# jenkinsm13/julia-spira

Measured on AMD Instinct MI355X. Metric: Msamples/sec at 1920x1080 spp=64 depth=8; fraction of HBM roofline, higher is better.
Workload: dtype f64

## Files before the change

include/spira_hip.h:

```cpp
#ifndef SPIRA_HIP_H
#define SPIRA_HIP_H

#include <stdint.h>

#ifdef __cplusplus
extern "C" {
#endif

#define SPIRA_ABI_VERSION 3

#define SPIRA_OK            0
#define SPIRA_E_INVALID    -1
#define SPIRA_E_NO_DEVICE  -2
#define SPIRA_E_HIP        -3
#define SPIRA_E_LIMIT      -4
#define SPIRA_E_UNSUPPORTED -5

#define SPIRA_SEM_MASK          0x0000000Fu
#define SPIRA_SEM_A             0x00000000u
#define SPIRA_SEM_CPU           0x00000001u
#define SPIRA_SEM_METAL         0x00000002u
#define SPIRA_SEM_HYBRID        0x00000003u
#define SPIRA_KERNEL_MASK       0x000000F0u
#define SPIRA_KERNEL_DEFAULT    0x00000000u
// ... 223 lines not shown
int spira_scene_radiance_f64(const spira_scene *scene, const double *rays6, uint32_t n_rays, const spira_radiance *rp,
                             double *sum_rgb, uint8_t *out_valid);
int spira_scene_radiance_device_f32(const spira_scene *scene, const float *d_rays6, uint32_t n_rays, const spira_radiance *rp,
                                    float *d_sum_rgb, uint8_t *d_out_valid, void *stream);
int spira_scene_radiance_device_f64(const spira_scene *scene, const double *d_rays6, uint32_t n_rays, const spira_radiance *rp,
                                    double *d_sum_rgb, uint8_t *d_out_valid, void *stream);

#define SPIRA_CAM_PINHOLE 0u
#define SPIRA_CAM_THIN_LENS 1u
#define SPIRA_CAM_ORTHO 2u
typedef struct spira_lens {
    uint32_t model, width, height, sample;
    uint64_t seed;
    uint32_t row0, rows;
    double   lens_radius;
} spira_lens;
int spira_camera_rays_f32(const float camera12[12], const spira_lens *lens, float *rays6);
int spira_camera_rays_f64(const double camera12[12], const spira_lens *lens, double *rays6);
int spira_camera_rays_device_f32(const float camera12[12], const spira_lens *lens, float *d_rays6, void *stream);
int spira_camera_rays_device_f64(const double camera12[12], const spira_lens *lens, double *d_rays6, void *stream);

typedef struct spira_gather_visible {
    uint32_t spp, sample0;
    uint64_t seed;
    uint32_t key0, flags;
    double   t_min, t_max;
} spira_gather_visible;
int spira_gather_rays_f32(const float *points6, uint32_t n_points, uint32_t sample, uint64_t seed, uint32_t key0, float *rays6);
int spira_gather_rays_f64(const double *points6, uint32_t n_points, uint32_t sample, uint64_t seed, uint32_t key0, double *rays6);
int spira_gather_rays_device_f32(const float *d_points6, uint32_t n_points, uint32_t sample, uint64_t seed, uint32_t key0, float *d_rays6, void *stream);
int spira_gather_rays_device_f64(const double *d_points6, uint32_t n_points, uint32_t sample, uint64_t seed, uint32_t key0, double *d_rays6, void *stream);
int spira_scene_gather_f32(const spira_scene *scene, const float *points6, uint32_t n_points, const spira_radiance *rp,
                           float *sum_rgb, uint8_t *out_valid);
int spira_scene_gather_f64(const spira_scene *scene, const double *points6, uint32_t n_points, const spira_radiance *rp,
                           double *sum_rgb, uint8_t *out_valid);
int spira_scene_gather_device_f32(const spira_scene *scene, const float *d_points6, uint32_t n_points, const spira_radiance *rp,
                                  float *d_sum_rgb, uint8_t *d_out_valid, void *stream);
int spira_scene_gather_device_f64(const spira_scene *scene, const double *d_points6, uint32_t n_points, const spira_radiance *rp,
                                  double *d_sum_rgb, uint8_t *d_out_valid, void *stream);
int spira_scene_gather_visible_f32(const spira_scene *scene, const float *points6, uint32_t n_points, const spira_gather_visible *gv,
                                   uint32_t *visible_u32, uint8_t *out_valid);
int spira_scene_gather_visible_f64(const spira_scene *scene, const double *points6, uint32_t n_points, const spira_gather_visible *gv,
                                   uint32_t *visible_u32, uint8_t *out_valid);
int spira_scene_gather_visible_device_f32(const spira_scene *scene, const float *d_points6, uint32_t n_points, const spira_gather_visible *gv,
                                          uint32_t *d_visible_u32, uint8_t *d_out_valid, void *stream);
int spira_scene_gather_visible_device_f64(const spira_scene *scene, const double *d_points6, uint32_t n_points, const spira_gather_visible *gv,
                                          uint32_t *d_visible_u32, uint8_t *d_out_valid, void *stream);

int spira_accumulate_f32(const float *spheres5, const float *materials8, const float *triangles10,
                         const float camera12[12], const spira_params *params, uint32_t sample0,
                         float *sum_rgb, uint32_t *rng_states);
int spira_accumulate_f64(const double *spheres5, const double *materials8, const double *triangles10,
                         const double camera12[12], const spira_params *params, uint32_t sample0,
                         double *sum_rgb, uint32_t *rng_states);
int spira_accumulate_device_f32(const float *spheres5, const float *materials8, const float *triangles10,
                                const float camera12[12], const spira_params *params, uint32_t sample0,
                                float *d_sum_rgb, uint32_t *d_rng_states, void *stream);
int spira_accumulate_device_f64(const double *spheres5, const double *materials8, const double *triangles10,
                                const double camera12[12], const spira_params *params, uint32_t sample0,
                                double *d_sum_rgb, uint32_t *d_rng_states, void *stream);

typedef struct spira_adaptive {
    uint32_t min_spp, batch_spp;
    double   tolerance, floor;
} spira_adaptive;
int spira_render_adaptive_f32(const float *spheres5, const float *materials8, const float *triangles10,
                              const float camera12[12], const spira_params *params, const spira_adaptive *adaptive,
                              float *out_hdr, float *out_img, uint32_t *out_spp, float *out_q);
int spira_render_adaptive_f64(const double *spheres5, const double *materials8, const double *triangles10,
                              const double camera12[12], const spira_params *params, const spira_adaptive *adaptive,
                              double *out_hdr, double *out_img, uint32_t *out_spp, double *out_q);
int spira_render_adaptive_scene_f32(const spira_scene *scene, const float camera12[12], const spira_params *params, const spira_adaptive *adaptive,
                                    float *out_hdr, float *out_img, uint32_t *out_spp, float *out_q);
int spira_render_adaptive_scene_f64(const spira_scene *scene, const double camera12[12], const spira_params *params, const spira_adaptive *adaptive,
                                    double *out_hdr, double *out_img, uint32_t *out_spp, double *out_q);
int spira_render_adaptive_scene_device_f32(const spira_scene *scene, const float camera12[12], const spira_params *params, const spira_adaptive *adaptive,
                                           float *d_out_hdr, float *d_out_img, uint32_t *d_out_spp, float *d_out_q, void *stream);
int spira_render_adaptive_scene_device_f64(const spira_scene *scene, const double camera12[12], const spira_params *params, const spira_adaptive *adaptive,
                                           double *d_out_hdr, double *d_out_img, uint32_t *d_out_spp, double *d_out_q, void *stream);
int spira_adaptive_converged_f32(const float sum3[3], float q, uint32_t n, double tolerance, double floor);
int spira_adaptive_converged_f64(const double sum3[3], double q, uint32_t n, double tolerance, double floor);

int spira_sky_pixel_f64(const double camera12[12], uint32_t width, uint32_t height, uint32_t i, uint32_t j, const double *spheres5, uint32_t n_spheres);

int spira_render_features_f32(const float *spheres5, const float *materials8, const float *triangles10,
                              const float camera12[12], const spira_params *params,
                              float *out_albedo, float *out_normal, float *out_depth);
int spira_render_features_f64(const double *spheres5, const double *materials8, const double *triangles10,
                              const double camera12[12], const spira_params *params,
                              double *out_albedo, double *out_normal, double *out_depth);
int spira_render_features_scene_f32(const spira_scene *scene, const float camera12[12], const spira_params *params,
                                    float *out_albedo, float *out_normal, float *out_depth);
int spira_render_features_scene_f64(const spira_scene *scene, const double camera12[12], const spira_params *params,
                                    double *out_albedo, double *out_normal, double *out_depth);
int spira_render_features_scene_device_f32(const spira_scene *scene, const float camera12[12], const spira_params *params,
                                           float *d_out_albedo, float *d_out_normal, float *d_out_depth, void *stream);
int spira_render_features_scene_device_f64(const spira_scene *scene, const double camera12[12], const spira_params *params,
                                           double *d_out_albedo, double *d_out_normal, double *d_out_depth, void *stream);

typedef struct spira_denoise {
    uint32_t width, height, iterations, post;
    double   sigma_l, sigma_z;
} spira_denoise;
int spira_denoise_f32(const float *color, const float *variance, const float *albedo, const float *normal, const float *depth,
                      const spira_denoise *dn, float *out_hdr, float *out_img);
int spira_denoise_f64(const double *color, const double *variance, const double *albedo, const double *normal, const double *depth,
                      const spira_denoise *dn, double *out_hdr, double *out_img);
int spira_denoise_device_f32(const float *d_color, const float *d_variance, const float *d_albedo, const float *d_normal, const float *d_depth,
                             const spira_denoise *dn, float *d_out_hdr, float *d_out_img, void *stream);
int spira_denoise_device_f64(const double *d_color, const double *d_variance, const double *d_albedo, const double *d_normal, const double *d_depth,
                             const spira_denoise *dn, double *d_out_hdr, double *d_out_img, void *stream);

int spira_trace_paths_f32(const float *spheres5, const float *materials8, const float *triangles10,
                          const float camera12[12], const spira_params *params, uint32_t n_paths,
                          const uint32_t *ijs, int *prims, float *ts, float *dirs, float *radiance);
int spira_trace_paths_f64(const double *spheres5, const double *materials8, const double *triangles10,
                          const double camera12[12], const spira_params *params, uint32_t n_paths,
                          const uint32_t *ijs, int *prims, double *ts, double *dirs, double *radiance);

int spira_tonemap_f32(float *values, uint64_t n, uint32_t post);

uint32_t spira_stripe_rows(uint32_t height, uint32_t stripe_h, uint32_t stripe_count, uint32_t stripe_rank);

#ifdef __cplusplus
}
#endif
#endif
```

julia-spira_amd/csrc/spira_device.h:

```cpp
#pragma once
#include <hip/hip_runtime.h>
#include <stdint.h>
#include <type_traits>
#include "spira_fastdiv.h"
#include "spira_sky.h"

namespace spira {

__device__ __forceinline__ float sqrt_rn(float x) { return __builtin_sqrtf(x); }
__device__ __forceinline__ double sqrt_rn(double x) { return __builtin_sqrt(x); }

constexpr int kBlock = 256;
#ifndef SPIRA_WAVES_F32
#define SPIRA_WAVES_F32 5
#endif
#ifndef SPIRA_WAVES_F64
#define SPIRA_WAVES_F64 4
#endif
#define SPIRA_WAVES_PER_SIMD(T) (sizeof(T) == 8 ? SPIRA_WAVES_F64 : SPIRA_WAVES_F32)
constexpr uint32_t kMaxTries = 64;

template <class T> struct Vec { T x, y, z; };

template <class T> __device__ __forceinline__ Vec<T> mk(T x, T y, T z) { Vec<T> r; r.x = x; r.y = y; r.z = z; return r; }
// ... 655 lines not shown
    asm volatile("" :: "v"(u0.x), "v"(u0.y), "v"(u0.z), "v"(u0.w), "v"(u1.x), "v"(u1.y), "v"(u1.z), "v"(u1.w), "v"(u2.x), "v"(u2.y), "v"(u2.z), "v"(u2.w) : "memory");
    if (do_tri) {
        float t_hi;
        const int cls = tri_screen_f32(u0, u1, u2, r, dx, dy, dz, t_hi);
        if (cls != 0) {
            w.c3 = w.c2; w.c2 = w.c1; w.c1 = w.c0; w.c0 = ti; ++w.nc;
            if (cls == 2) r.best = __builtin_fminf(r.best, t_hi);
        }
    }
    if (do_node) {
        uint32_t ih, lh;
        bvh8_node(n0, n1, n2, n3, n4, r, ih, lh);
        w.G = (n1.x << 8) | ih;
        w.tw = n1.y | (lh << 24);
        w.rank = n1.z;
    }
    return ((w.tw >> 24) != 0 || (w.G & 0xFFu) != 0 || w.sp > 0) ? kWalkOn : kWalkDone;
}

template <class T, int KL = 0>
__device__ __forceinline__ void bvh_closest_hit(const SceneLds<T> &sc, Vec<T> o, Vec<T> d, T t_min, T &closest, int &prim, uint32_t &slot, uint32_t *lds_stack = nullptr) {
    Bvh8Ray r; T t0;
    if (!bvh8_enter<T>(sc, o, d, closest, r, t0)) return;
    Bvh8Walk<T> w;
    bvh8_begin<T>(w, r, t0, t_min, sc.bvh_root[2].w);
    uint32_t stack[kBvhStackD - KL];
    const uint32_t lane = threadIdx.x & 63;
    const int base = (int)(sc.n_spheres + sc.n_triangles);
    while (bvh8_step<T, KL>(sc, w, r, o, d, t_min, base, closest, prim, slot, lds_stack, stack, lane)) {}
    while (w.nc) bvh8_resolve_one<T>(sc, w, r, o, d, t_min, base, closest, prim, slot);
}

template <class T, class P, bool TRI = true, bool CAM = false>
__device__ __forceinline__ void closest_hit_local(const SceneLds<T> &sc, Vec<T> o, Vec<T> d, T t_min, T &closest, int &prim, P &pol, const Pack4<T> *cam = nullptr) {
    closest = (T)INFINITY;
    prim = -1;
    const T a = dot(d, d);
    const T two_a = (T)2.0 * a;
    const T four_a = (T)4 * a;
    const RootDiv<T> over_2a = root_divisor<T>(two_a, pol);
    root_t_min<T>(t_min, pol);
    const Pack4<T> *sph = CAM ? cam : sc.sph;
    Pack4<T> c_next = sph[0];
#pragma unroll 2
    for (uint32_t s = 0; s < sc.n_spheres; ++s) {
        const Pack4<T> c = c_next;
        c_next = sph[s + 1 < sc.n_spheres ? s + 1 : s];
        Vec<T> oc; T cc;
        if (CAM) { oc = mk<T>(c.x, c.y, c.z); cc = c.w; }
        else {
            oc = o - mk<T>(c.x, c.y, c.z);
            cc = dot(oc, oc) - c.w;
        }
        T b = (T)2.0 * dot(oc, d);
        const T bb = b * b;
        T disc = bb - four_a * cc;
        if (!(disc < 0)) {
            root_operands<T>(bb, disc, pol);
            T sq = root_sqrt<T>(disc, pol);
            T root = root_over<T>(-b - sq, over_2a, pol);
            bool ok = !(root < t_min || root > closest);
            if (!ok && root < t_min) {
                root = root_over<T>(-b + sq, over_2a, pol);
                ok = !(root < t_min || root > closest);
            }
            if (ok) { closest = root; prim = (int)s; }
        }
    }
    if (TRI && sc.n_triangles) {
        Pack4<T> v0n = sc.tri[0], e1n = sc.tri[1], e2n = sc.tri[2];
#pragma unroll 2
        for (uint32_t i = 0; i < sc.n_triangles; ++i) {
            const Pack4<T> v0 = v0n, e1 = e1n, e2 = e2n;
            const uint32_t nx = i + 1 < sc.n_triangles ? i + 1 : i;
            v0n = sc.tri[3 * nx]; e1n = sc.tri[3 * nx + 1]; e2n = sc.tri[3 * nx + 2];
            T t;
            if (triangle_test<T>(v0, e1, e2, o, d, t_min, closest, t, pol)) {
                closest = t; prim = (int)(sc.n_spheres + i);
            }
        }
    }
}

template <class T>
__device__ __forceinline__ bool mesh_box_hit(const SceneLds<T> &sc, Vec<T> o, Vec<T> d, T closest) {
    const Vec<T> inv = mk<T>(rcp_fast(d.x), rcp_fast(d.y), rcp_fast(d.z));
    return box_entry<T>(sc.bvh_root[0], sc.bvh_root[1], o, inv, closest) >= (T)0;
}

template <class T>
__device__ __forceinline__ void closest_hit_local(const SceneLds<T> &sc, Vec<T> o, Vec<T> d, T t_min, T &closest, int &prim) {
    ExactDiv exact;
    closest_hit_local<T>(sc, o, d, t_min, closest, prim, exact);
}
template <class T, bool BVH, class P, bool TRI = true>
__device__ __forceinline__ int closest_hit(const SceneLds<T> &sc, Vec<T> o, Vec<T> d, T t_min, T &t_hit, uint32_t &slot, P &pol) {
    T closest; int prim;
    closest_hit_local<T, P, TRI>(sc, o, d, t_min, closest, prim, pol);
    slot = 0;
    if (BVH) bvh_closest_hit<T>(sc, o, d, t_min, closest, prim, slot);
    t_hit = closest;
    return prim;
}
template <class T, bool BVH>
__device__ __forceinline__ int closest_hit(const SceneLds<T> &sc, Vec<T> o, Vec<T> d, T t_min, T &t_hit, uint32_t &slot) {
    ExactDiv exact;
    return closest_hit<T, BVH>(sc, o, d, t_min, t_hit, slot, exact);
}

template <class T> __device__ __forceinline__ Vec<T> random_in_unit_sphere(const RngKey &k) {
    Vec<T> p = mk<T>(0, 0, 0);
    for (uint32_t t = 1; t <= kMaxTries; ++t) {
        T u0, u1, u2;
        rng3<T>(k, t, u0, u1, u2, (T)(1.0 / 1048576.0));
        Vec<T> q = mk<T>(u0, u1, u2) - mk<T>(1, 1, 1);
        if (dot(q, q) < (T)1.0) { p = q; break; }
    }
    return p;
}

enum : uint32_t { kDead = 0, kDiffuse = 1, kSpecRough = 2, kMirror = 3, kDielectric = 4 };
template <class T> struct Pending { Vec<T> v; T rough; uint32_t kind; };
struct SegInfo { int prim; bool alive; bool has_contrib; };

template <class T> struct ExtState {
    uint32_t flags;
    T bR, bG, bB;
};

template <class T> __device__ __forceinline__ T spd_lookup(const T *tab, int row, int i, T f) {
    const T *t = tab + row * kSpdN;
    return t[i] + (t[i + 1] - t[i]) * f;
}
template <class T>
__device__ __forceinline__ Vec<T> ext_wavelength(const SceneLds<T> &sc, uint32_t sA, uint32_t sB, uint32_t pixel, uint32_t sample, ExtState<T> &ext) {
    T xu, xv, u2;
    rng3<T>(rng_key(sA, sB, pixel, sample, 0), 0, xu, xv, u2);
    const T x = u2 * (T)(kSpdN - 1);
    int i = (int)x;
    i = i > kSpdN - 2 ? kSpdN - 2 : i;
    const T f = x - (T)i;
    ext.bR = spd_lookup<T>(sc.spd, 0, i, f); ext.bG = spd_lookup<T>(sc.spd, 1, i, f); ext.bB = spd_lookup<T>(sc.spd, 2, i, f);
    return mk<T>(spd_lookup<T>(sc.spd, 3, i, f), spd_lookup<T>(sc.spd, 4, i, f), spd_lookup<T>(sc.spd, 5, i, f));
}
template <class T> __device__ __forceinline__ T ext_uplift(const ExtState<T> &ext, const Vec<T> c) { return (c.x * ext.bR + c.y * ext.bG) + c.z * ext.bB; }

template <class T> __device__ __forceinline__ Vec<T> sky_term(const Vec<T> d, const Vec<T> beta) {
    T ts = (T)0.5 * (d.y + (T)1.0);
    Vec<T> sky = mk<T>(1.0, 1.0, 1.0) * ((T)1.0 - ts) + mk<T>((T)0.5, (T)0.7, (T)1.0) * ts;
    return mulv(beta, sky);
}
template <class T, bool EXT> __device__ __forceinline__ Vec<T> sky_term_x(const Vec<T> d, const Vec<T> beta, const ExtState<T> *ext) {
    if (EXT && (ext->flags & kExtSpectral)) {
        T ts = (T)0.5 * (d.y + (T)1.0);
        Vec<T> sky = mk<T>(1.0, 1.0, 1.0) * ((T)1.0 - ts) + mk<T>((T)0.5, (T)0.7, (T)1.0) * ts;
        return beta * ext_uplift<T>(*ext, sky);
    }
    return sky_term<T>(d, beta);
}

template <class T, bool BVH, bool TRI = true> __device__ __forceinline__ int material_of(const SceneLds<T> &sc, int prim, uint32_t slot) {
    if ((!TRI && !BVH) || prim < (int)sc.n_spheres) return sc.smat[prim];
    if (TRI && (!BVH || prim < (int)(sc.n_spheres + sc.n_triangles))) return sc.tmat[prim - (int)sc.n_spheres];
    return (int)Bits<T>::to_u32(sc.bvh_tris[3 * (size_t)slot + 1].w);
}

// ... 76 lines not shown
    int prim = closest_hit<T, BVH>(sc, o, d, (T)0.001, t, slot);
    info.prim = prim;
    t_out = prim >= 0 ? t : (T)0;
    if (prim < 0) {
        pend.kind = kDead; pend.rough = 0; pend.v = mk<T>(0, 0, 0);
        contrib = sky_term_x<T, EXT>(d, beta, ext);
        info.alive = false; info.has_contrib = true;
        return info;
    }
    const Vec<T> pos = o + d * t;
    info.has_contrib = shade_hit<T, BVH, EXT>(sc, pos, d, prim, slot, beta, scatter, contrib, pend, ext);
    info.alive = scatter;
    if (scatter) o = pos;
    return info;
}

template <class T, class P>
__device__ __forceinline__ Vec<T> segment_back(const Vec<T> pos, const Pending<T> &pend, const Vec<T> rnd, P &pol) {
    if (pend.kind == kDiffuse) return normalize((pend.v + rnd) - pos, pol);
    Vec<T> reflected = pend.v;
    if (pend.kind == kSpecRough) reflected = reflected + rnd * pend.rough;
    return normalize(reflected, pol);
}
template <class T>
__device__ __forceinline__ Vec<T> segment_back(const Vec<T> pos, const Pending<T> &pend, const Vec<T> rnd) {
    ExactDiv exact;
    return segment_back<T>(pos, pend, rnd, exact);
}

template <class T, bool BVH, bool EXT = false>
__device__ __forceinline__ SegInfo trace_segment(const SceneLds<T> &sc, const RenderConst<T> &rc, Vec<T> &o, Vec<T> &d,
                                                 Vec<T> &beta, uint32_t pixel, uint32_t sample, uint32_t bounce,
                                                 bool scatter, Vec<T> &contrib, T &t_out, const ExtState<T> *ext = nullptr) {
    Pending<T> pend;
    const Vec<T> d_in = d;
    SegInfo info = segment_front<T, BVH, EXT>(sc, o, d, beta, scatter, contrib, t_out, pend, ext);
    if (info.alive) {
        Vec<T> rnd = mk<T>(0, 0, 0);
        if (EXT && pend.kind == kDielectric) dielectric_resolve<T>(pend, d_in, rng_key(rc.sA, rc.sB, pixel, sample, bounce));
        if (pend.kind == kDiffuse || pend.kind == kSpecRough)
            rnd = random_in_unit_sphere<T>(rng_key(rc.sA, rc.sB, pixel, sample, bounce));
        d = segment_back<T>(o, pend, rnd);
    }
    return info;
}

template <class T, class P>
__device__ __forceinline__ void camera_ray(const RenderConst<T> &rc, uint32_t i, uint32_t j, uint32_t pixel, uint32_t sample,
                                           Vec<T> &o, Vec<T> &d, P &pol) {
    T xu, xv, unused;
    rng3<T>(rng_key(rc.sA, rc.sB, pixel, sample, 0), 0, xu, xv, unused);
    T u = ((T)(i - 1) + xu) / (T)(rc.width - 1);
    T v = ((T)(j - 1) + xv) / (T)(rc.height - 1);
    o = rc.cam_origin;
    d = normalize(((rc.cam_llc + rc.cam_hor * u) + rc.cam_ver * v) - o, pol);
}
template <class T>
__device__ __forceinline__ void camera_ray(const RenderConst<T> &rc, uint32_t i, uint32_t j, uint32_t pixel, uint32_t sample,
                                           Vec<T> &o, Vec<T> &d) {
    ExactDiv exact;
    camera_ray<T>(rc, i, j, pixel, sample, o, d, exact);
}
__device__ __forceinline__ float to_scalar(float x) { return __uint_as_float(__builtin_amdgcn_readfirstlane(__float_as_uint(x))); }
__device__ __forceinline__ double to_scalar(double x) {
    const uint32_t lo = __builtin_amdgcn_readfirstlane((uint32_t)__double2loint(x)), hi = __builtin_amdgcn_readfirstlane((uint32_t)__double2hiint(x));
    return __hiloint2double((int)hi, (int)lo);
}
template <class T> struct PixelDiv { Recip<T> w1, h1; };
template <class T> __device__ __forceinline__ PixelDiv<T> pixel_divisors(const RenderConst<T> &rc) {
    PixelDiv<T> p;
    p.w1 = recip_of((T)(rc.width - 1)); p.h1 = recip_of((T)(rc.height - 1));
    p.w1.d = to_scalar(p.w1.d); p.w1.r = to_scalar(p.w1.r); p.h1.d = to_scalar(p.h1.d); p.h1.r = to_scalar(p.h1.r);
    return p;
}
template <class T> __device__ __forceinline__ T pixel_quotient(T n, const Recip<T> &rc, ExactDiv &) { return n / rc.d; }
template <class T> __device__ __forceinline__ T pixel_quotient(T n, const Recip<T> &rc, SpecDiv &) { return quotient(n, rc); }
template <class T, class P>
__device__ __forceinline__ void camera_ray_lds(const RenderConst<T> &rc, const T *cam, const PixelDiv<T> &pd, uint32_t i, uint32_t j, uint32_t pixel, uint32_t sample,
                                               Vec<T> &o, Vec<T> &d, P &pol) {
    T xu, xv, unused;
    rng3<T>(rng_key(rc.sA, rc.sB, pixel, sample, 0), 0, xu, xv, unused);
    T u = pixel_quotient<T>((T)(i - 1) + xu, pd.w1, pol);
    T v = pixel_quotient<T>((T)(j - 1) + xv, pd.h1, pol);
    o = mk<T>(cam[0], cam[1], cam[2]);
    const Vec<T> llc = mk<T>(cam[3], cam[4], cam[5]), hor = mk<T>(cam[6], cam[7], cam[8]), ver = mk<T>(cam[9], cam[10], cam[11]);
    d = normalize(((llc + hor * u) + ver * v) - o, pol);
}

template <class T>
__device__ __forceinline__ void path_of(const RenderConst<T> &rc, uint32_t q, uint32_t pass, uint32_t &i, uint32_t &j,
                                        uint32_t &pixel, uint32_t &sample) {
    uint32_t slot = fastdiv(q, rc.fd_tile);
    uint32_t pl = q - slot * rc.tile_pixels;
    uint32_t lr = fastdiv(pl, rc.fd_width);
    uint32_t lx = pl - lr * rc.width;
    j = ref_row_j(rc, lr);
    i = lx + 1;
    pixel = (j - 1) * rc.width + lx;
    sample = rc.sample0 + pass * rc.slots + slot;
}

template <class T> struct RayQueue { Pack4<T> *A; Pack4<T> *B; Pack2<T> *C; };

struct Stats {
    unsigned long long segments, rays_enqueued, radiance_rmw, radiance_store, redone_waves, rays_parked;
    unsigned long long mesh_wave_trips, mesh_lane_trips;
    unsigned long long sky_pixels;
};

template <class T> struct BounceArgs {
    SceneGlobal<T> scene;
    RenderConst<T> rc;
    RayQueue<T> qin, qout;
    Pack3<T> *L;
    const uint32_t *cnt_in;
    uint32_t *cnt_out;
    uint32_t *blk_stats;
    uint32_t cap;
    Stats *stats;
    uint32_t bounce;
    uint32_t pass;
    uint32_t n_first;
};

__device__ __forceinline__ void wave_lds_sync() {
    __builtin_amdgcn_fence(__ATOMIC_RELEASE, "wavefront");
    __builtin_amdgcn_wave_barrier();
    __builtin_amdgcn_fence(__ATOMIC_ACQUIRE, "wavefront");
}

#ifndef SPIRA_RND_TAIL
#define SPIRA_RND_TAIL 1
#endif
#ifndef SPIRA_RND_INT
#define SPIRA_RND_INT 1
#endif
template <class T> constexpr bool kRndPacked = SPIRA_RND_INT && sizeof(T) == 8;

template <class T, bool PACKED = kRndPacked<T>> struct RndTry {
    Vec<T> c;
    __device__ __forceinline__ bool draw(const RngKey &k, uint32_t t) {
        T u0, u1, u2;
        rng3<T>(k, t, u0, u1, u2, (T)(1.0 / 1048576.0));
        c = mk<T>(u0, u1, u2) - mk<T>(1, 1, 1);
        return dot(c, c) < (T)1.0;
    }
    __device__ __forceinline__ void zero() { c = mk<T>(0, 0, 0); }
    __device__ __forceinline__ void store(Pack4<T> *slot) const { Pack4<T> w; w.x = c.x; w.y = c.y; w.z = c.z; w.w = 0; *slot = w; }
    static __device__ __forceinline__ Vec<T> load(const Pack4<T> *slot) { const Pack4<T> w = *slot; return mk<T>(w.x, w.y, w.z); }
};
template <class T> struct RndTry<T, true> {
    uint32_t a, b;
    __device__ __forceinline__ bool draw(const RngKey &k, uint32_t t) {
        a = mix32((k.hA + t * 0x9E3779B9u) ^ k.hBr);
        b = mix32(a + k.hB);
        const int32_t k0 = (int32_t)(a >> 11) - (1 << 20), k1 = (int32_t)(b >> 11) - (1 << 20);
        const int32_t k2 = (int32_t)(((a & 0x7FFu) << 10) | (b & 0x3FFu)) - (1 << 20);
        const uint64_t s = (uint64_t)((int64_t)k0 * k0) + (uint64_t)((int64_t)k1 * k1) + (uint64_t)((int64_t)k2 * k2);
        return s < (1ull << 40);
    }
    __device__ __forceinline__ void zero() { a = 0x80000400u; b = 0x80000000u; }
    __device__ __forceinline__ void store(Pack4<T> *slot) const { *reinterpret_cast<uint2 *>(slot) = make_uint2(a, b); }
    static __device__ __forceinline__ Vec<T> load(const Pack4<T> *slot) {
        const uint2 w = *reinterpret_cast<const uint2 *>(slot);
        const T s = (T)(1.0 / 1048576.0);
        const T u0 = (T)(w.x >> 11) * s, u1 = (T)(w.y >> 11) * s, u2 = (T)(((w.x & 0x7FFu) << 10) | (w.y & 0x3FFu)) * s;
// ... 145 lines not shown
                    q[r] |= 0x80000000u;
                } else if (!si.alive && !has_l) {
                    Pack3<T> l; l.x = 0; l.y = 0; l.z = 0;
                    a.L[qi] = l;
                    ++n_store;
                }
                want = (pend[r].kind == kDiffuse || pend[r].kind == kSpecRough);
                if (want) {
                    if (!FIRST) path_of<T>(rc, qi, a.pass, pi, pj, pixel, sample);
                    key = rng_key(rc.sA, rc.sB, pixel, sample, a.bounce);
                }
            }
            if (scatter) {
                const unsigned long long m = __ballot(want);
                if (want) {
                    ent[r] = n_list + __popcll(m & lt_mask);
                    uint32_t *kw = reinterpret_cast<uint32_t *>(&s_rnd[ent[r]]);
                    kw[0] = key.hA; kw[1] = key.hB;
                }
                n_list += (uint32_t)__popcll(m);
            }
        }
        if (!scatter) continue;
        wave_lds_sync();
        drain_unit_sphere_list<T>(s_rnd, n_list, lane);
        wave_lds_sync();
#pragma unroll
        for (int r = 0; r < R; ++r) {
            const bool alive = pend[r].kind != kDead;
            const unsigned long long m = __ballot(alive);
            if (alive) {
                Vec<T> rnd = mk<T>(0, 0, 0);
                if (pend[r].kind != kMirror) rnd = RndTry<T>::load(&s_rnd[ent[r]]);
                const Vec<T> nd = segment_back<T>(o[r], pend[r], rnd);
                const uint32_t dst = region + fill + __popcll(m & lt_mask);
                Pack4<T> A, B; Pack2<T> C;
                A.x = o[r].x; A.y = o[r].y; A.z = o[r].z; A.w = nd.x;
                B.x = nd.y; B.y = nd.z; B.z = beta[r].x; B.w = beta[r].y;
                C.x = beta[r].z; C.y = Bits<T>::from_u32(q[r]);
                a.qout.A[dst] = A; a.qout.B[dst] = B; a.qout.C[dst] = C;
            }
            fill += (uint32_t)__popcll(m);
        }
        wave_lds_sync();
    }
    for (int sft = 32; sft > 0; sft >>= 1) { n_rmw += __shfl_down(n_rmw, sft); n_seg += __shfl_down(n_seg, sft); n_store += __shfl_down(n_store, sft); }
    if (lane == 0) {
        if (scatter) a.cnt_out[wid] = fill;
        a.blk_stats[4 * wid] = n_seg;
        a.blk_stats[4 * wid + 1] = n_rmw;
        a.blk_stats[4 * wid + 2] = n_store;
        a.blk_stats[4 * wid + 3] = FIRST ? 0u : n_seg;
    }
}

template <class T> struct PathArgs {
    SceneGlobal<T> scene;
    RenderConst<T> rc;
    RayQueue<T> q[2];
    uint32_t *qref[2];
    uint2 *qkey[2];
    uint32_t cam_consts;
    Pack3<T> *L;
    uint32_t *blk_stats;
    uint32_t cap;
    uint32_t pass;
    uint32_t n_first;
    uint32_t dense_pct;
    Pack4<T> *mesh_list;
    uint32_t mesh_min_batch;
    uint32_t refill_free;
    uint32_t mesh_mode;
    uint32_t *mesh_count;
    uint32_t resume_k, resume_nw;
    uint32_t *redo;
    uint32_t redo_only;
    Stats *stats;
    Pack4<T> *accum;
    FastDiv fd_keff;
    uint32_t k_eff;
    uint32_t accum_first;
    uint32_t l_private;
    uint32_t sky_runs;
};

#ifndef SPIRA_RESOLVE_RUN
#define SPIRA_RESOLVE_RUN 4
#endif
__device__ __forceinline__ uint32_t owned_pixel(uint32_t w, uint32_t nw, uint32_t l) {
    constexpr uint32_t kRun = SPIRA_RESOLVE_RUN;
    static_assert(64 % kRun == 0, "a run length divides the wave");
    return ((l / kRun) * nw + w) * kRun + l % kRun;
}

template <class T>
__device__ __forceinline__ void resolve_pixel(Pack4<T> *accum, const Pack3<T> *L, uint32_t tile_pixels, uint32_t k_eff, bool first_pass, uint32_t p) {
    Pack4<T> acc;
    if (first_pass) { acc.x = 0; acc.y = 0; acc.z = 0; acc.w = 0; } else acc = accum[p];
    uint32_t s = 0;
    for (; s + 8 <= k_eff; s += 8) {
        Pack3<T> l[8];
#pragma unroll
        for (int k = 0; k < 8; ++k) l[k] = L[(size_t)(s + k) * tile_pixels + p];
#pragma unroll
        for (int k = 0; k < 8; ++k) { acc.x = acc.x + l[k].x; acc.y = acc.y + l[k].y; acc.z = acc.z + l[k].z; }
    }
    for (; s < k_eff; ++s) {
        const Pack3<T> l = L[(size_t)s * tile_pixels + p];
        acc.x = acc.x + l.x; acc.y = acc.y + l.y; acc.z = acc.z + l.z;
    }
    accum[p] = acc;
}
template <class T>
__device__ __forceinline__ void resolve_pixel_run(Pack4<T> *accum, const Pack3<T> *Lp, uint32_t k_eff, bool first_pass, uint32_t p) {
    constexpr uint32_t kRun = SPIRA_RESOLVE_RUN;
    Pack4<T> acc;
    if (first_pass) { acc.x = 0; acc.y = 0; acc.z = 0; acc.w = 0; } else acc = accum[p];
    uint32_t s = 0;
    for (; s + 8 <= k_eff; s += 8) {
        Pack3<T> l[8];
#pragma unroll
        for (int k = 0; k < 8; ++k) l[k] = Lp[(s + k) * kRun];
#pragma unroll
        for (int k = 0; k < 8; ++k) { acc.x = acc.x + l[k].x; acc.y = acc.y + l[k].y; acc.z = acc.z + l[k].z; }
    }
    for (; s < k_eff; ++s) {
        const Pack3<T> l = Lp[s * kRun];
        acc.x = acc.x + l.x; acc.y = acc.y + l.y; acc.z = acc.z + l.z;
    }
    accum[p] = acc;
}

__device__ __forceinline__ float pack_qref(uint32_t q, uint32_t, float) { return __uint_as_float(q); }
__device__ __forceinline__ double pack_qref(uint32_t q, uint32_t ref, double) { return __longlong_as_double((long long)((unsigned long long)q | ((unsigned long long)ref << 32))); }
__device__ __forceinline__ uint32_t unpack_q(float w) { return __float_as_uint(w); }
__device__ __forceinline__ uint32_t unpack_q(double w) { return (uint32_t)(unsigned long long)__double_as_longlong(w); }
__device__ __forceinline__ uint32_t unpack_ref(double w) { return (uint32_t)((unsigned long long)__double_as_longlong(w) >> 32); }

#ifdef SPIRA_MESH_STATS
__device__ unsigned long long g_mesh_dbg[32];
#define MESH_STAT(...) __VA_ARGS__
#else
#define MESH_STAT(...)
#endif

#ifndef SPIRA_CARRY_KEY
#define SPIRA_CARRY_KEY 1
#endif
#ifndef SPIRA_WAVES_B_F32
#define SPIRA_WAVES_B_F32 4
#endif
#ifndef SPIRA_WAVES_B_F64
#define SPIRA_WAVES_B_F64 SPIRA_WAVES_F64
#endif
#ifndef SPIRA_WAVES_PATH_F32
#define SPIRA_WAVES_PATH_F32 6
#endif
template <class T, int R, bool BVH, bool EXT, bool SPEC, int MODE = 0, bool TRI = true>
__global__ __launch_bounds__(kBlock, MODE == 2 ? (sizeof(T) == 8 ? SPIRA_WAVES_B_F64 : SPIRA_WAVES_B_F32) : (sizeof(T) == 4 ? SPIRA_WAVES_PATH_F32 : SPIRA_WAVES_F64)) void k_path(const PathArgs<T> a) {
    extern __shared__ __attribute__((aligned(32))) unsigned char lds_raw[];
    constexpr uint32_t WPB = kBlock / 64, SUB = 64 * R;
    constexpr bool kRefArray = sizeof(T) == 4;
    constexpr bool kCarry = SPIRA_CARRY_KEY && !BVH && !EXT;
    constexpr uint32_t kStageShift = 25, kRefMask = (1u << kStageShift) - 1u;
    const uint32_t lane = threadIdx.x & 63, wave = threadIdx.x >> 6;
    const uint32_t NW = gridDim.x * WPB, wid = blockIdx.x * WPB + wave;
    const RenderConst<T> &rc = a.rc;
    using Pol = typename std::conditional<SPEC, SpecDiv, ExactDiv>::type;
    Pol pol;
    if (!SPEC && a.redo_only) {
        uint32_t any = 0;
        for (uint32_t w = 0; w < WPB; ++w) any |= a.redo[blockIdx.x * WPB + w];
        if (!any) return;
    }
    T *cam_lds = reinterpret_cast<T *>(lds_raw + scene_lds_bytes<T>(a.scene.n_spheres, a.scene.n_materials, a.scene.n_triangles) + WPB * SUB * sizeof(Pack4<T>));
    if (threadIdx.x < 12) {
        const Vec<T> *cv = threadIdx.x < 3 ? &rc.cam_origin : (threadIdx.x < 6 ? &rc.cam_llc : (threadIdx.x < 9 ? &rc.cam_hor : &rc.cam_ver));
        const uint32_t cc = threadIdx.x % 3;
        cam_lds[threadIdx.x] = cc == 0 ? cv->x : (cc == 1 ? cv->y : cv->z);
    }
    Pack4<T> *cam_sph = reinterpret_cast<Pack4<T> *>(reinterpret_cast<unsigned char *>(cam_lds) + 128);
    constexpr bool kCam = !EXT;
    if (kCam && MODE != 2 && a.cam_consts)
        for (uint32_t i = threadIdx.x; i < a.scene.n_spheres; i += blockDim.x) {
            const T *sp = a.scene.spheres5 + 5 * (size_t)i;
            const Vec<T> oc = rc.cam_origin - mk<T>(sp[0], sp[1], sp[2]);
            Pack4<T> k; k.x = oc.x; k.y = oc.y; k.z = oc.z; k.w = dot(oc, oc) - sp[3] * sp[3];
            cam_sph[i] = k;
        }
    const SceneLds<T> sc = stage_scene<T>(a.scene, lds_raw);
    const PixelDiv<T> pix_div = pixel_divisors<T>(rc);
    if (!SPEC && a.redo_only) {
        if (!a.redo[wid]) return;
        if (lane == 0) atomicAdd(&a.stats->redone_waves, 1ull);
    }
    Pack4<T> *s_rnd = reinterpret_cast<Pack4<T> *>(lds_raw + scene_lds_bytes<T>(a.scene.n_spheres, a.scene.n_materials, a.scene.n_triangles)) + wave * SUB;
    constexpr uint32_t mesh_mode = BVH ? (uint32_t)MODE : 0u;
    const uint32_t kseg = mesh_mode == 2u ? a.resume_k : 1u;
    if (mesh_mode == 2u && wid * kseg >= a.resume_nw) return;
    const uint32_t region = wid * kseg * a.cap;
    const unsigned long long lt_mask = (1ull << lane) - 1ull;
    const uint32_t ref_base = sc.n_spheres + sc.n_triangles;
    const bool mixed = mesh_mode != 0u || rc.max_depth <= 128u;
    const uint32_t dense_pct = mixed ? a.dense_pct : 0u;
    const bool defer = mesh_mode != 0u || (BVH && mixed && a.mesh_list != nullptr);
    Pack4<T> *mlist = a.mesh_list + 3 * (size_t)region;
    uint32_t n_rmw = 0, n_store = 0, n_seg = 0, n_enq = 0, n_park = 0;
    uint32_t n_wtrips = 0, n_ltrips = 0;
    uint32_t n_in = 0;
    const bool own = !BVH && !EXT && !TRI && sizeof(T) == 8 && a.accum != nullptr;
    const uint32_t n_own = own ? 64u * a.k_eff : 0u;
    const uint32_t n_sub_first = own ? (n_own + SUB - 1) / SUB : (a.n_first + SUB - 1) / SUB;
    const bool priv = kCarry && own && a.l_private != 0;
    const uint32_t l_base = priv ? wid * n_own : 0u;
    constexpr bool kOwnT = !BVH && !EXT && !TRI && sizeof(T) == 8;
    uint32_t sky_mask = 0;
    uint32_t *sky_word = reinterpret_cast<uint32_t *>(cam_lds + 12) + wave;
    static_assert(12 * sizeof(T) + WPB * sizeof(uint32_t) <= 128 || !kOwnT, "a word per wave behind the camera");
    if constexpr (kOwnT) {
        if (own && a.sky_runs) {
            constexpr uint32_t kRun = SPIRA_RESOLVE_RUN, kRuns = 64 / kRun, kRowSlots = 64 / kRun;
            static_assert(kRun == 4 && 2 * 64 * sizeof(Pack3<T>) <= SUB * sizeof(Pack4<T>), "the run mask below is written for runs of 4; a row of terms fits the work list");
            {
                const uint32_t px = owned_pixel(wid, NW, lane);
                bool sky = false;
                if (px < rc.tile_pixels) {
                    uint32_t pi, pj, pixel, sample;
                    path_of<T>(rc, px, a.pass, pi, pj, pixel, sample);
                    sky = sky_pixel(cam_lds, rc.width, rc.height, pi, pj, a.scene.spheres5, a.scene.n_spheres);
                }
                unsigned long long b = __ballot(sky);
                b &= b >> 1; b &= b >> 2;
                for (uint32_t g = 0; g < kRuns; ++g) sky_mask |= (uint32_t)((b >> (kRun * g)) & 1ull) << g;
            }
            Pack3<T> *s_sky = reinterpret_cast<Pack3<T> *>(s_rnd);
            for (uint32_t m = sky_mask; m; m &= m - 1u) {
                const uint32_t g = (uint32_t)__builtin_ctz(m);
                const uint32_t px = owned_pixel(wid, NW, g * kRun + lane % kRun);
                uint32_t pi, pj, pixel, sample0;
                path_of<T>(rc, px, a.pass, pi, pj, pixel, sample0);
                Pack3<T> acc;
                acc.x = 0; acc.y = 0; acc.z = 0;
                if (!a.accum_first && lane < kRun) { const Pack4<T> a0 = a.accum[px]; acc.x = a0.x; acc.y = a0.y; acc.z = a0.z; }
                for (uint32_t s0 = 0; s0 < a.k_eff; s0 += kRowSlots) {
                    const uint32_t slot = s0 + lane / kRun;
                    if (slot < a.k_eff) {
                        Vec<T> o_, d_;
                        camera_ray_lds<T>(rc, cam_lds, pix_div, pi, pj, pixel, sample0 + slot, o_, d_, pol);
                        const Vec<T> c = sky_term_x<T, EXT>(d_, mk<T>(1, 1, 1), nullptr);
                        Pack3<T> l; l.x = c.x; l.y = c.y; l.z = c.z;
                        s_sky[lane] = l;
                        ++n_seg; ++n_store;
                    }
                    wave_lds_sync();
                    if (lane < kRun) {
                        const uint32_t n = a.k_eff - s0 < kRowSlots ? a.k_eff - s0 : kRowSlots;
                        for (uint32_t k = 0; k < n; ++k) { const Pack3<T> l = s_sky[k * kRun + lane]; acc.x = acc.x + l.x; acc.y = acc.y + l.y; acc.z = acc.z + l.z; }
                    }
                    wave_lds_sync();
                }
                if (lane < kRun) a.L[priv ? l_base + g * a.k_eff * kRun + lane : px] = acc;
            }
        }
        if (own) { if (lane == 0) *sky_word = sky_mask; wave_lds_sync(); }
    }

    auto park = [&](uint32_t slot_i, const Vec<T> o_, const Vec<T> d_, const Vec<T> beta_, T closest_, uint32_t q_, int prim_, uint32_t stage_hit) {
        Pack4<T> A, B, C;
        A.x = o_.x; A.y = o_.y; A.z = o_.z; A.w = d_.x;
        B.x = d_.y; B.y = d_.z; B.z = beta_.x; B.w = beta_.y;
        C.x = beta_.z; C.y = closest_; C.z = Bits<T>::from_u32(q_); C.w = Bits<T>::from_u32((uint32_t)(prim_ + 1) | (stage_hit << kStageShift));
        mlist[3 * (size_t)slot_i] = A; mlist[3 * (size_t)slot_i + 1] = B; mlist[3 * (size_t)slot_i + 2] = C;
    };
    uint32_t mfill = 0;
    constexpr int kMaxSeg = 16;
    uint32_t pfx[kMaxSeg + 1];
    bool segmented = false;
    {
        uint32_t cnt = 0;
        if (mesh_mode == 2u && lane < kseg && wid * kseg + lane < a.resume_nw) cnt = a.mesh_count[wid * kseg + lane];
        pfx[0] = 0;
#pragma unroll
        for (int j = 0; j < kMaxSeg; ++j) pfx[j + 1] = pfx[j] + (uint32_t)__builtin_amdgcn_readlane((int)cnt, j);
        if (mesh_mode == 2u) { mfill = pfx[kMaxSeg]; segmented = true; }
    }
    const uint32_t first_sub = own ? 0u : (mesh_mode == 1u ? (wid % a.resume_k) * (NW / a.resume_k) + wid / a.resume_k : wid);
    const uint32_t sub_step = own ? 1u : NW;
    MESH_STAT(unsigned long long dbg_t0 = __builtin_readcyclecounter(); unsigned long long dbg_sess = 0, dbg_walk = 0; uint32_t dbg_ns = 0, dbg_ws = 0, dbg_ls = 0, dbg_rf = 0, dbg_rays = 0, dbg_rounds = 0, dbg_ws1 = 0, dbg_ls1 = 0, dbg_h[4] = {0, 0, 0, 0};)
    for (uint32_t round = 0; ; ++round) {
        MESH_STAT(++dbg_rounds;)
        const bool first = mesh_mode != 2u && round == 0;
        const RayQueue<T> qin = a.q[(round + 1) & 1], qout = a.q[round & 1];
        const uint32_t *rin = a.qref[(round + 1) & 1];
        uint32_t *rout = a.qref[round & 1];
        const uint2 *kin = a.qkey[(round + 1) & 1];
        uint2 *kout = a.qkey[round & 1];
        const uint32_t limit = first ? (own ? n_own : a.n_first) : n_in;
        const uint32_t n_sub = first ? n_sub_first : (n_in + SUB - 1) / SUB;
        uint32_t fill = 0;
        for (uint32_t sub = first ? first_sub : 0u; sub < n_sub; sub += first ? sub_step : 1u) {
            if constexpr (kOwnT) if (own && first) {
                const uint32_t m = (uint32_t)__builtin_amdgcn_readfirstlane((int)*sky_word);
                const uint32_t r0 = fastdiv(sub * SUB / SPIRA_RESOLVE_RUN, a.fd_keff), r1 = fastdiv((sub * SUB + SUB - 1) / SPIRA_RESOLVE_RUN, a.fd_keff);
                if (r0 == r1 && ((m >> r0) & 1u)) continue;
            }
            Vec<T> o[R], beta[R];
            Pending<T> pend[R];
            ExtState<T> ex[R];
            uint32_t q[R], ent[R], stg[R], ref[R];
            uint32_t ka[R], kb[R];
            bool valid[R];
#pragma unroll
            for (int r = 0; r < R; ++r) {
                const uint32_t idx = sub * SUB + r * 64 + lane;
                valid[r] = false; stg[r] = round; ref[r] = 0; q[r] = 0; ka[r] = 0; kb[r] = 0;
                pend[r].kind = kDead; pend[r].rough = 0; pend[r].v = mk<T>(0, 0, 0);
                o[r] = mk<T>(0, 0, 0); beta[r] = mk<T>(1, 1, 1);
                bool parked = false; T park_t = 0; int park_prim = -1;
                uint32_t qf = idx;
                bool in = idx < limit;
                if (own && first) {
                    const uint32_t t = idx / SPIRA_RESOLVE_RUN, run = fastdiv(t, a.fd_keff);
                    const uint32_t px = owned_pixel(wid, NW, run * SPIRA_RESOLVE_RUN + idx % SPIRA_RESOLVE_RUN);
                    qf = (t - run * a.k_eff) * rc.tile_pixels + px;
                    in = in && px < rc.tile_pixels;
                    if constexpr (kOwnT) in = in && !((*sky_word >> run) & 1u);
                }
                const uint32_t ql = priv ? l_base + idx : qf;
                if (in) {
                    if (first) {
                        uint32_t pixel, sample, pi, pj;
                        Vec<T> d;
                        q[r] = ql;
                        path_of<T>(rc, qf, a.pass, pi, pj, pixel, sample);
                        if (kCarry) { ka[r] = mix32(rc.sA + pixel) ^ (sample << 8); kb[r] = mix32(rc.sB ^ pixel) + (sample << 8); }
                        camera_ray_lds<T>(rc, cam_lds, pix_div, pi, pj, pixel, sample, o[r], d, pol);
                        if (EXT) { ex[r].flags = rc.flags; if (rc.flags & kExtSpectral) beta[r] = ext_wavelength<T>(sc, rc.sA, rc.sB, pixel, sample, ex[r]); }
                        T t; uint32_t slot = 0;
                        int prim;
                        if (defer) {
                            if (kCam && a.cam_consts) closest_hit_local<T, Pol, TRI, true>(sc, o[r], d, (T)0.001, t, prim, pol, cam_sph);
                            else closest_hit_local<T, Pol, TRI>(sc, o[r], d, (T)0.001, t, prim, pol);
                            parked = mesh_box_hit<T>(sc, o[r], d, t);
                        } else if (kCam && !BVH && a.cam_consts) { closest_hit_local<T, Pol, TRI, true>(sc, o[r], d, (T)0.001, t, prim, pol, cam_sph); }
                        else prim = closest_hit<T, BVH, Pol, TRI>(sc, o[r], d, (T)0.001, t, slot, pol);
                        ++n_seg;
                        if (parked) { park_t = t; park_prim = prim; pend[r].v = d; }
                        else if (prim < 0) {
                            const Vec<T> c = sky_term_x<T, EXT>(d, beta[r], &ex[r]);
                            Pack3<T> l; l.x = c.x; l.y = c.y; l.z = c.z;
                            a.L[ql] = l;
                            ++n_store;
                        } else {
                            valid[r] = true;
                            o[r] = o[r] + d * t;
                            ref[r] = (BVH && prim >= (int)ref_base) ? ref_base + slot : (uint32_t)prim;
                            pend[r].v = d;
                        }
                    } else {
                        const Pack4<T> A = qin.A[region + idx], B = qin.B[region + idx];
                        const Pack2<T> C = qin.C[region + idx];
                        o[r] = mk<T>(A.x, A.y, A.z);
                        pend[r].v = mk<T>(A.w, B.x, B.y);
                        beta[r] = mk<T>(B.z, B.w, C.x);
                        q[r] = unpack_q(C.y);
                        uint32_t w;
                        if constexpr (kRefArray) w = rin[region + idx]; else w = unpack_ref(C.y);
                        if (mixed) { stg[r] = w >> kStageShift; ref[r] = w & kRefMask; } else ref[r] = w;
                        if (kCarry) { const uint2 k = kin[region + idx]; ka[r] = k.x; kb[r] = k.y; }
                        valid[r] = true;
                    }
                }
                if (defer && first) {
                    const unsigned long long mp = __ballot(parked);
                    if (parked) park(mfill + __popcll(mp & lt_mask), o[r], pend[r].v, beta[r], park_t, q[r], park_prim, 0u);
                    mfill += (uint32_t)__popcll(mp); n_park += (uint32_t)__popcll(mp);
                }
            }
            while (true) {
                uint32_t n_list = 0, n_valid = 0;
#pragma unroll
                for (int r = 0; r < R; ++r) {
                    bool want = false;
                    RngKey key;
                    const Vec<T> d = pend[r].v;
                    pend[r].kind = kDead;
                    if (valid[r]) {
                        uint32_t pixel = 0, sample = 0, pi, pj;
                        const bool scatter = stg[r] + 1 < rc.max_depth;
                        int prim = (int)ref[r]; uint32_t slot = 0;
                        if (BVH && ref[r] >= ref_base) { prim = (int)ref_base; slot = ref[r] - ref_base; }
                        const uint32_t qi = q[r] & 0x7FFFFFFFu;
                        const bool has_l = (q[r] >> 31) != 0;
                        if (EXT) {
                            path_of<T>(rc, qi, a.pass, pi, pj, pixel, sample);
                            ex[r].flags = rc.flags;
                            if (rc.flags & kExtSpectral) (void)ext_wavelength<T>(sc, rc.sA, rc.sB, pixel, sample, ex[r]);
                        }
                        Vec<T> contrib;
                        const bool has_contrib = shade_hit<T, BVH, EXT, Pol, TRI>(sc, o[r], d, prim, slot, beta[r], scatter, contrib, pend[r], &ex[r], pol);
                        if (has_contrib) {
                            Pack3<T> l; l.x = contrib.x; l.y = contrib.y; l.z = contrib.z;
                            if (has_l) { const Pack3<T> l0 = a.L[qi]; l.x = l0.x + contrib.x; l.y = l0.y + contrib.y; l.z = l0.z + contrib.z; ++n_rmw; }
                            else ++n_store;
                            a.L[qi] = l;
                            q[r] |= 0x80000000u;
                        } else if (!scatter && !has_l) {
                            Pack3<T> l; l.x = 0; l.y = 0; l.z = 0;
                            a.L[qi] = l;
                            ++n_store;
                        }
                        want = (pend[r].kind == kDiffuse || pend[r].kind == kSpecRough);
                        if (want || (EXT && pend[r].kind == kDielectric)) {
                            if (kCarry && mixed) {
                                key.hA = mix32(ka[r] ^ stg[r]); key.hB = mix32(kb[r] + stg[r]); key.hBr = (key.hB << 16) | (key.hB >> 16);
                            } else {
                                if (!EXT) path_of<T>(rc, qi, a.pass, pi, pj, pixel, sample);
                                key = rng_key(rc.sA, rc.sB, pixel, sample, stg[r]);
                            }
                            if (EXT && pend[r].kind == kDielectric) dielectric_resolve<T>(pend[r], d, key);
                        }
                    }
                    const unsigned long long mv = __ballot(pend[r].kind != kDead);
                    n_valid += (uint32_t)__popcll(mv);
                    const unsigned long long m = __ballot(want);
                    if (want) {
                        ent[r] = n_list + __popcll(m & lt_mask);
// ... 228 lines not shown
                        const Vec<T> hp = o_ + d_ * closest;
                        const uint32_t w_ = ((prim >= (int)ref_base) ? ref_base + slot : (uint32_t)prim) | (stage_hit << kStageShift);
                        const uint32_t dst = region + fill + __popcll(mh & lt_mask);
                        Pack4<T> A, B; Pack2<T> C;
                        A.x = hp.x; A.y = hp.y; A.z = hp.z; A.w = d_.x;
                        B.x = d_.y; B.y = d_.z; B.z = beta_.x; B.w = beta_.y;
                        C.x = beta_.z; C.y = pack_qref(q_, w_, (T)0);
                        qout.A[dst] = A; qout.B[dst] = B; qout.C[dst] = C;
                        if constexpr (kRefArray) rout[dst] = w_;
                    }
                }
                fill += (uint32_t)__popcll(mh);
                finished = false;
                const unsigned long long mf = __ballot(!walking);
                const uint32_t take = min((uint32_t)__popcll(mf), mfill - next);
                if (!walking && (uint32_t)__popcll(mf & lt_mask) < take) {
                    const uint32_t e = next + (uint32_t)__popcll(mf & lt_mask);
                    const Pack4<T> *ent = mlist + 3 * (size_t)e;
                    if (segmented) {
                        uint32_t seg = 0, off = e;
#pragma unroll
                        for (int j = 1; j < kMaxSeg; ++j) if (e >= pfx[j]) { seg = (uint32_t)j; off = e - pfx[j]; }
                        ent = a.mesh_list + 3 * ((size_t)(wid * kseg + seg) * a.cap + off);
                    }
                    const Pack4<T> A = ent[0], B = ent[1], C = ent[2];
                    o_ = mk<T>(A.x, A.y, A.z); d_ = mk<T>(A.w, B.x, B.y); beta_ = mk<T>(B.z, B.w, C.x);
                    closest = C.y;
                    q_ = Bits<T>::to_u32(C.z);
                    const uint32_t pw = Bits<T>::to_u32(C.w);
                    prim = (int)(pw & kRefMask) - 1;
                    stage_hit = pw >> kStageShift;
                    slot = 0;
                    T t0;
                    if (bvh8_enter<T>(sc, o_, d_, closest, ry, t0)) { bvh8_begin<T>(wk, ry, t0, (T)0.001, sc.bvh_root[2].w); walking = true; }
                    else finished = true;
                }
                next += take;
                if (!__any(walking)) { if (__any(finished)) continue; break; }
                const bool more = next < mfill;
                MESH_STAT(++dbg_rf; const unsigned long long dbg_w0 = __builtin_readcyclecounter();)
                uint32_t n_now = (uint32_t)__popcll(__ballot(walking));
                while (true) {
                    ++n_wtrips; n_ltrips += n_now;
                    MESH_STAT(++dbg_ws; { const uint32_t nl = (uint32_t)__popcll(__ballot(walking)); dbg_ls += nl; if (segmented) { ++dbg_ws1; dbg_ls1 += nl; } ++dbg_h[nl <= 8 ? 0 : (nl <= 24 ? 1 : (nl <= 48 ? 2 : 3))]; })
                    if (walking && !bvh8_step<T, kLdsStack>(sc, wk, ry, o_, d_, (T)0.001, (int)ref_base, closest, prim, slot, lstack, stack, lane)) { walking = false; finished = true; }
                    const uint32_t n_walk = (uint32_t)__popcll(__ballot(walking));
                    n_now = n_walk;
                    if (n_walk == 0 || (more && 64u - n_walk >= a.refill_free)) break;
                }

                MESH_STAT(dbg_walk += __builtin_readcyclecounter() - dbg_w0;)
            }
            }
            mfill = 0;
            segmented = false;
            MESH_STAT(dbg_sess += __builtin_readcyclecounter() - dbg_s0;)
        }
        n_in = fill;
        n_enq += fill;
        if (n_in == 0 && (mfill == 0 || mesh_mode == 1u)) break;
        __builtin_amdgcn_fence(__ATOMIC_RELEASE, "workgroup");
        __builtin_amdgcn_fence(__ATOMIC_ACQUIRE, "workgroup");
    }
    for (int sft = 32; sft > 0; sft >>= 1) { n_rmw += __shfl_down(n_rmw, sft); n_seg += __shfl_down(n_seg, sft); n_store += __shfl_down(n_store, sft); }
    const bool again = SPEC && __any(outside_window<T>(pol));
    if (own && !again && !(SPEC && a.redo_only == 2u)) {
        __builtin_amdgcn_fence(__ATOMIC_RELEASE, "workgroup");
        __builtin_amdgcn_fence(__ATOMIC_ACQUIRE, "workgroup");
        const uint32_t px = owned_pixel(wid, NW, lane);
        bool summed = false;
        if constexpr (kOwnT) sky_mask = (uint32_t)__builtin_amdgcn_readfirstlane((int)*sky_word);
        if constexpr (kOwnT) summed = ((sky_mask >> (lane / SPIRA_RESOLVE_RUN)) & 1u) != 0;
        if (summed) {
            const Pack3<T> l = a.L[priv ? l_base + (lane / SPIRA_RESOLVE_RUN) * a.k_eff * SPIRA_RESOLVE_RUN + lane % SPIRA_RESOLVE_RUN : px];
            Pack4<T> acc;
            if (a.accum_first) acc.w = 0; else acc = a.accum[px];
            acc.x = l.x; acc.y = l.y; acc.z = l.z;
            a.accum[px] = acc;
        } else if (px < rc.tile_pixels) {
            if (priv) resolve_pixel_run<T>(a.accum, a.L + l_base + (lane / SPIRA_RESOLVE_RUN) * a.k_eff * SPIRA_RESOLVE_RUN + lane % SPIRA_RESOLVE_RUN, a.k_eff, a.accum_first != 0, px);
            else resolve_pixel<T>(a.accum, a.L, rc.tile_pixels, a.k_eff, a.accum_first != 0, px);
        }
        const uint32_t seg = __shfl(n_seg, 0), rmw = __shfl(n_rmw, 0), sto = __shfl(n_store, 0);
        if (lane < 4) {
            unsigned long long *f = lane == 0 ? &a.stats->segments : (lane == 1 ? &a.stats->rays_enqueued : (lane == 2 ? &a.stats->radiance_rmw : &a.stats->radiance_store));
            atomicAdd(f, (unsigned long long)(lane == 0 ? seg : (lane == 1 ? n_enq : (lane == 2 ? rmw : sto))));
        }
        if constexpr (kOwnT) if (lane == 4 && sky_mask) atomicAdd(&a.stats->sky_pixels, (unsigned long long)(SPIRA_RESOLVE_RUN * __popc(sky_mask)));
    }
    MESH_STAT(if (lane == 0) { unsigned long long *g = g_mesh_dbg + (mesh_mode == 2u ? 16 : 0);
                               atomicAdd(&g[0], __builtin_readcyclecounter() - dbg_t0); atomicAdd(&g[1], dbg_sess); atomicAdd(&g[2], (unsigned long long)dbg_ns);
                               atomicAdd(&g[3], (unsigned long long)dbg_ws); atomicAdd(&g[4], (unsigned long long)dbg_ls); atomicAdd(&g[5], (unsigned long long)dbg_rf);
                               atomicAdd(&g[6], (unsigned long long)dbg_rays); atomicAdd(&g[7], (unsigned long long)dbg_rounds); atomicAdd(&g[9], dbg_walk); atomicAdd(&g[10], 1ull); atomicAdd(&g[11], (unsigned long long)dbg_ws1); atomicAdd(&g[12], (unsigned long long)dbg_ls1);
                               atomicAdd(&g[8], (unsigned long long)dbg_h[0]); atomicAdd(&g[13], (unsigned long long)dbg_h[1]); atomicAdd(&g[14], (unsigned long long)dbg_h[2]); atomicAdd(&g[15], (unsigned long long)dbg_h[3]); })
    if (lane == 0) {
        if (mesh_mode == 2u) {
            const uint32_t row = 4 * wid * kseg;
            a.blk_stats[row] += n_seg; a.blk_stats[row + 1] += n_rmw; a.blk_stats[row + 2] += n_store; a.blk_stats[row + 3] += n_enq;
        } else {
            a.blk_stats[4 * wid] = n_seg;
            a.blk_stats[4 * wid + 1] = n_rmw;
            a.blk_stats[4 * wid + 2] = n_store;
            a.blk_stats[4 * wid + 3] = n_enq;
            if (mesh_mode == 1u) a.mesh_count[wid] = mfill;
        }
        if (SPEC) a.redo[wid] = again ? 1u : 0u;
        if (BVH && n_park && !again && !(SPEC && a.redo_only == 2u)) atomicAdd(&a.stats->rays_parked, (unsigned long long)n_park);
        if (BVH && mesh_mode != 1u && n_wtrips && !again && !(SPEC && a.redo_only == 2u)) { atomicAdd(&a.stats->mesh_wave_trips, (unsigned long long)n_wtrips); atomicAdd(&a.stats->mesh_lane_trips, (unsigned long long)n_ltrips); }
    }
}

template <class T, bool BVH, bool EXT>
__global__ __launch_bounds__(kBlock) void k_mega(const BounceArgs<T> a) {
    extern __shared__ __attribute__((aligned(32))) unsigned char lds_raw[];
    const SceneLds<T> sc = stage_scene<T>(a.scene, lds_raw);
    const RenderConst<T> &rc = a.rc;
    unsigned long long nseg = 0;
    const uint32_t stride = gridDim.x * kBlock;
    uint32_t idx = blockIdx.x * kBlock + threadIdx.x;
    bool fresh = true;
    uint32_t pixel = 0, sample = 0, b = 0;
    Vec<T> o = mk<T>(0, 0, 0), d = mk<T>(0, 0, 1), beta = mk<T>(1, 1, 1), Lacc = mk<T>(0, 0, 0);
    ExtState<T> ex; ex.flags = rc.flags; ex.bR = 0; ex.bG = 0; ex.bB = 0;
    while (idx < a.n_first) {
        if (fresh) {
            uint32_t pi, pj;
            path_of<T>(rc, idx, a.pass, pi, pj, pixel, sample);
            camera_ray<T>(rc, pi, pj, pixel, sample, o, d);
            beta = mk<T>(1, 1, 1); Lacc = mk<T>(0, 0, 0); b = 0;
            if (EXT && (rc.flags & kExtSpectral)) beta = ext_wavelength<T>(sc, rc.sA, rc.sB, pixel, sample, ex);
            fresh = false;
        }
        Vec<T> contrib; T t_hit;
        SegInfo si = trace_segment<T, BVH, EXT>(sc, rc, o, d, beta, pixel, sample, b, b + 1 < rc.max_depth, contrib, t_hit, &ex);
        ++nseg;
        if (b == 0) { if (si.has_contrib) Lacc = contrib; }
        else if (si.has_contrib) Lacc = Lacc + contrib;
        ++b;
        if (!si.alive || b == rc.max_depth) {
            Pack3<T> l; l.x = Lacc.x; l.y = Lacc.y; l.z = Lacc.z;
            a.L[idx] = l;
            idx += stride;
            fresh = true;
        }
    }
    for (int sft = 32; sft > 0; sft >>= 1) nseg += __shfl_down(nseg, sft);
    if ((threadIdx.x & 63) == 0 && nseg) atomicAdd(&a.stats->segments, nseg);
}

template <class T, bool BVH, bool EXT>
__global__ __launch_bounds__(64) void k_trace(const BounceArgs<T> a, const uint32_t *ijs, uint32_t n_paths, int *prims, T *ts,
                                              T *dirs, T *radiance) {
    extern __shared__ __attribute__((aligned(32))) unsigned char lds_raw[];
    const SceneLds<T> sc = stage_scene<T>(a.scene, lds_raw);
    const RenderConst<T> &rc = a.rc;
    uint32_t p = blockIdx.x * blockDim.x + threadIdx.x;
    if (p >= n_paths) return;
    uint32_t i = ijs[3 * p], j = ijs[3 * p + 1], sample = ijs[3 * p + 2];
    uint32_t pixel = (j - 1) * rc.width + (i - 1);
    Vec<T> o, d, beta = mk<T>(1, 1, 1), Lacc = mk<T>(0, 0, 0);
    camera_ray<T>(rc, i, j, pixel, sample, o, d);
    ExtState<T> ex; ex.flags = rc.flags; ex.bR = 0; ex.bG = 0; ex.bB = 0;
    if (EXT && (rc.flags & kExtSpectral)) beta = ext_wavelength<T>(sc, rc.sA, rc.sB, pixel, sample, ex);
    for (uint32_t b = 0; b < rc.max_depth; ++b) {
        Vec<T> contrib; T t_hit;
        Vec<T> dir_in = d;
        SegInfo si = trace_segment<T, BVH, EXT>(sc, rc, o, d, beta, pixel, sample, b, b + 1 < rc.max_depth, contrib, t_hit, &ex);
        size_t k = (size_t)p * rc.max_depth + b;
        prims[k] = si.prim; ts[k] = t_hit;
        dirs[3 * k] = dir_in.x; dirs[3 * k + 1] = dir_in.y; dirs[3 * k + 2] = dir_in.z;
        if (b == 0) { if (si.has_contrib) Lacc = contrib; }
// ... 756 lines not shown
```

julia-spira_amd/csrc/spira_hip.hip:

```cpp
#include <hip/hip_runtime.h>
#include <sys/mman.h>
#include <rccl/rccl.h>
#include <dlfcn.h>

#include <algorithm>
#include <atomic>
#include <chrono>
#include <cmath>
#include <cstdio>
#include <cstdlib>
#include <cstring>
#include <condition_variable>
#include <mutex>
#include <new>
#include <string>
#include <thread>
#include <type_traits>
#include <vector>

#include "../../include/spira_hip.h"
#include "../../include/spira_spd.h"
#include "spira_device.h"
#include "spira_bvh.h"
#include "spira_validate.h"
// ... 584 lines not shown
                std::memcpy(pieces[i].dst, (const char *)c.h_stage + pieces[i].off, pieces[i].len);
            }
        };
        std::vector<std::thread> thr;
        for (int t = 1; t < n_thr; ++t) thr.emplace_back(mover, t);
        mover(0);
        for (auto &t : thr) t.join();
        for (hipError_t e : errs) if (e != hipSuccess) return e;
        return hipSuccess;
    }
};

int copy_out(Ctx &c, hipStream_t st, void *const dst[2], const void *const src[2], size_t bytes_each) {
    const size_t kChunk = (size_t)std::max<uint32_t>(1, env_u32("SPIRA_STAGE_CHUNK_MB", 8)) << 20, kMinStaged = 4u << 20, kMaxStaged = 512u << 20;
    const int n_out = (dst[0] ? 1 : 0) + (dst[1] ? 1 : 0);
    if (!n_out) return 0;
    const size_t total = bytes_each * (size_t)n_out;
    if (bytes_each < kMinStaged || total > kMaxStaged || !stage_reserve(c, total)) {
        for (int k = 0; k < 2; ++k) if (dst[k]) HIP_TRY(hipMemcpyAsync(dst[k], src[k], bytes_each, hipMemcpyDeviceToHost, st));
        return 0;
    }
    StagedCopy sc(c);
    for (int k = 0; k < 2; ++k)
        for (size_t o = 0; dst[k] && o < bytes_each; o += kChunk)
            HIP_TRY(sc.stage(st, (char *)dst[k] + o, (const char *)src[k] + o, std::min(kChunk, bytes_each - o)));
    const hipError_t e = sc.move();
    if (e != hipSuccess) return fail(SPIRA_E_HIP, std::string("copy_out: ") + hipGetErrorString(e));
    return 0;
}

template <class T>
int acquire_scene(Ctx &c, hipStream_t st, const spira_scene *h, const T *spheres5, const T *materials8, const T *triangles10,
                  const spira_params *p, spira::SceneGlobal<T> &g, bool reuse = false) {
    if (h) { scene_pointers<T>(h->store, g); return 0; }
    if (reuse) { scene_pointers<T>(c.scene, g); return 0; }
    const uint32_t nt = triangles10 ? p->n_triangles : 0;
    if (int rc = scene_upload<T>(c.scene, st, c.have_done ? c.ev_done : nullptr, spheres5, materials8, triangles10, p->n_spheres, p->n_materials, nt)) return rc;
    scene_pointers<T>(c.scene, g);
    return 0;
}

template <class T>
int attach_spd(Ctx &c, hipStream_t st, uint32_t flags, spira::SceneGlobal<T> &g) {
    g.spd = nullptr;
    if (!(flags & SPIRA_EXT_SPECTRAL)) return 0;
    DevBuf &b = sizeof(T) == 4 ? c.spd32 : c.spd64;
    if (!b.p) {
        static_assert(SPIRA_SPD_N == spira::kSpdN && SPIRA_SPD_ROWS == spira::kSpdRows, "SPD table shape");
        T host[SPIRA_SPD_ROWS * SPIRA_SPD_N];
        for (int r = 0; r < SPIRA_SPD_ROWS; ++r)
            for (int i = 0; i < SPIRA_SPD_N; ++i) host[r * SPIRA_SPD_N + i] = (T)spira_spd_table[r][i];
        if (int rc = b.ensure(sizeof host)) return rc;
        HIP_TRY(hipMemcpy(b.p, host, sizeof host, hipMemcpyHostToDevice));
    }
    (void)st;
    g.spd = (const T *)b.p;
    return 0;
}
template <class T>
int attach_spd(Ctx &c, hipStream_t st, const spira_params *p, spira::SceneGlobal<T> &g) { return attach_spd<T>(c, st, p->flags, g); }

template <class T>
int check_handle(const spira_scene *h) {
    if (!h || h->magic != kSceneMagic) return fail(SPIRA_E_INVALID, "scene handle is NULL or was destroyed");
    if (h->prec != (int)sizeof(T)) return fail(SPIRA_E_INVALID, "scene handle was created in the other precision");
    if (h->device != tl_device) return fail(SPIRA_E_INVALID, "scene handle belongs to another device (spira_set_device)");
    return 0;
}

spira::Knobs read_knobs() {
    spira::Knobs k;
    k.batch_rays = env_u32("SPIRA_BATCH_RAYS", k.batch_rays);
    k.R = env_u32("SPIRA_R", k.R);
    k.blocks_per_cu = env_u32("SPIRA_BLOCKS_PER_CU", 0);
    k.defer_mesh = env_u32("SPIRA_DEFER_MESH", 1); k.mesh_two_pass = env_u32("SPIRA_MESH_TWO_PASS", 1);
    k.fused_resolve = env_u32("SPIRA_FUSED_RESOLVE", 1); k.private_l = env_u32("SPIRA_PRIVATE_L", 1);
    k.spec_div = env_u32("SPIRA_SPEC_DIV", 1);
    k.dense_pct = std::min<uint32_t>(env_u32("SPIRA_DENSE_PCT", 70), 100);
    k.mesh_min_batch = std::max<uint32_t>(1, env_u32("SPIRA_MESH_MIN_BATCH", 128));
    k.mesh_refill = std::min<uint32_t>(64, std::max<uint32_t>(1, env_u32("SPIRA_MESH_REFILL", 16)));
    k.mesh_fat_waves_per_cu = env_u32("SPIRA_MESH_FAT_WAVES_PER_CU", 16);
    k.cam_consts = env_u32("SPIRA_CAM_CONSTS", 1);
    k.sky_runs = env_u32("SPIRA_SKY_RUNS", 1);
    return k;
}
template <class T>
spira::PlanIn plan_input(const Ctx &c, const spira_params *p, uint32_t rows, uint32_t nt_scene, bool progressive, bool caller_rng, bool out_on_device) {
    spira::PlanIn in;
    in.width = p->width; in.rows = rows; in.spp = p->spp; in.max_depth = p->max_depth; in.flags = p->flags; in.batch_rays = p->batch_rays;
    in.n_triangles = nt_scene; in.num_cus = (uint32_t)c.num_cus;
    in.progressive = progressive; in.caller_rng = caller_rng; in.out_on_device = out_on_device;
    in.prec = sizeof(T); in.block = spira::kBlock; in.waves_per_simd = SPIRA_WAVES_PER_SIMD(T); in.carry_key = SPIRA_CARRY_KEY;
    in.pack4 = sizeof(spira::Pack4<T>); in.pack3 = sizeof(spira::Pack3<T>); in.pack2 = sizeof(spira::Pack2<T>);
    in.k = read_knobs();
    return in;
}

int ensure_workspaces(Ctx &c, const spira::Workspace &w) {
    for (int i = 0; i < 2; ++i) {
        if (int rc = c.qA[i].ensure(w.queue4)) return rc;
        if (int rc = c.qB[i].ensure(w.queue4)) return rc;
        if (int rc = c.qC[i].ensure(w.queue2)) return rc;
        if (int rc = c.qR[i].ensure(w.q_ref)) return rc;
        if (int rc = c.qK[i].ensure(w.q_key)) return rc;
        if (int rc = c.qX[i].ensure(w.q_x)) return rc;
    }
    const struct { DevBuf &b; uint64_t bytes; } rest[] = {
        {c.mesh_list, w.mesh_list}, {c.mesh_count, w.mesh_count}, {c.redo, w.redo}, {c.blkstats, w.blkstats}, {c.L, w.L}, {c.counts, w.counts},
        {c.stats, sizeof(spira::Stats)}, {c.accum, w.accum}, {c.out_tmp, w.out_tmp}, {c.rng, w.rng},
        {c.hyb_state, w.hyb_state}, {c.hyb_mat, w.hyb_mat}, {c.hyb_flags, w.hyb_flags}};
    for (const auto &r : rest)
        if (int rc = r.b.ensure(r.bytes)) return rc;
    return 0;
}

template <class T>
int verify_path_args(const Ctx &c, const spira::PathArgs<T> &a, uint32_t first_launch_blocks) {
    using P4 = spira::Pack4<T>;
    using P2 = spira::Pack2<T>;
    spira::PathLaunch l;
    l.blocks = first_launch_blocks; l.cap = a.cap; l.n_first = a.n_first; l.k_eff = a.k_eff;
    l.tile_pixels = a.rc.tile_pixels; l.max_depth = a.rc.max_depth; l.flags = a.rc.flags; l.n_lds_triangles = a.scene.n_triangles;
    l.mesh_mode = a.mesh_mode; l.resume_k = a.resume_k; l.resume_nw = a.resume_nw;
    l.mesh = a.scene.n_bvh_tris != 0; l.pixel_owning = a.accum != nullptr; l.l_private = a.l_private != 0;
    l.prec = sizeof(T); l.wpb = spira::kBlock / 64; l.carry_key = SPIRA_CARRY_KEY;
    const spira::PathNeed need = spira::path_need(l);
    const uint64_t nw = need.nw, n = need.packets;
    auto covers = [](const DevBuf &b, const void *ptr, uint64_t bytes) { return ptr == b.p && b.p != nullptr && b.cap >= bytes; };
    const char *bad = need.fits ? nullptr : "the pass does not fit its queue regions";
    if (a.rc.max_depth > 1 || l.mesh)
        for (int i = 0; i < 2 && !bad; ++i) {
            if (!covers(c.qA[i], a.q[i].A, n * sizeof(P4)) || !covers(c.qB[i], a.q[i].B, n * sizeof(P4)) || !covers(c.qC[i], a.q[i].C, n * sizeof(P2))) bad = "hit queues";
            else if (sizeof(T) == 4 && !covers(c.qR[i], a.qref[i], n * sizeof(uint32_t))) bad = "hit reference arrays";
            else if (!l.mesh && !covers(c.qK[i], a.qkey[i], n * sizeof(uint2))) bad = "carried RNG keys";
        }
    if (!bad && a.mesh_list && !covers(c.mesh_list, a.mesh_list, 3 * n * sizeof(P4))) bad = "mesh lists";
    if (!bad && a.mesh_mode != 0 && (!a.mesh_list || !covers(c.mesh_count, a.mesh_count, nw * sizeof(uint32_t)) || !need.resume_ok)) bad = "parked-ray counts of a two-launch mesh pass";
    if (!bad && a.redo && !covers(c.redo, a.redo, nw * sizeof(uint32_t))) bad = "redo flags";
    if (!bad && !covers(c.blkstats, a.blk_stats, nw * 4 * sizeof(uint32_t))) bad = "per-wave statistics";
    if (!bad && !covers(c.L, a.L, need.l_entries * sizeof(spira::Pack3<T>))) bad = "per-path radiance";
    if (!bad && !covers(c.stats, a.stats, sizeof(spira::Stats))) bad = "counters";
    if (!bad && a.accum && (!covers(c.accum, a.accum, (uint64_t)a.rc.tile_pixels * sizeof(P4)) || !need.owning_ok)) bad = "pixel-owning pass";
    if (!bad && a.l_private && !need.private_ok) bad = "wave-private radiance blocks";
    if (bad) return fail(SPIRA_E_LIMIT, std::string("internal: a workspace is smaller than the launch needs (") + bad + ")");
    return 0;
}

template <class T>
int validate_call(const spira_scene *h, const T *spheres5, const T *materials8, const T *triangles10, const T *camera12, const spira_params *p,
                  const T *out_hdr, const T *out_img, bool progressive, uint32_t sample0, const uint32_t *rng_states, uint32_t *rows) {
    if (!p) return fail(SPIRA_E_INVALID, "params is NULL");
    const uint32_t nt = triangles10 ? p->n_triangles : 0;
    if (h) { if (int rc = check_handle<T>(h)) return rc; }
    else if (int rc = validate_scene<T>(spheres5, materials8, triangles10, p->n_spheres, p->n_materials, nt)) return rc;
    if (int rc = validate_params(camera12, p, h ? h->store.nt : nt, rows)) return rc;
    if (!out_hdr && !out_img) return fail(SPIRA_E_INVALID, "both outputs are NULL");
    const char *msg = nullptr;
    if (int rc = spira::sample_range_check(progressive, sample0, p->spp, &msg)) return fail(rc, msg);
    if (progressive && (p->flags & SPIRA_SEM_MASK) == SPIRA_SEM_HYBRID) return fail(SPIRA_E_UNSUPPORTED, "SPIRA_SEM_HYBRID has no accumulate entry (its image is a mean of tone-mapped samples)");
    if (progressive && (p->flags & SPIRA_SEM_MASK) == SPIRA_SEM_METAL && sample0 > 0 && !rng_states)
        return fail(SPIRA_E_INVALID, "SPIRA_SEM_METAL with sample0 > 0 needs rng_states (the LCG states the previous call left); "
                                     "without them every call would replay the samples of the first");
    return 0;
}

template <class T> struct Call {
    Ctx &c;
    hipStream_t st;
    const spira_params *p;
    const spira::Plan &plan;
    spira::BounceArgs<T> a{};
    size_t lds = 0;
    int spec = 0;
    bool progressive = false, profile = false;
    uint32_t sample0 = 0, *d_rng = nullptr;
    uint64_t launches = 0, metal_launches = 0;
    using P4 = spira::Pack4<T>;
    using P2 = spira::Pack2<T>;
    P4 *accum() const { return (P4 *)c.accum.p; }
    spira::Stats *stats() const { return (spira::Stats *)c.stats.p; }
    uint32_t *redo() const { return (uint32_t *)c.redo.p; }
    spira::RayQueue<T> queue(int i) const { return {(P4 *)c.qA[i].p, (P4 *)c.qB[i].p, (P2 *)c.qC[i].p}; }
    dim3 block() const { return dim3(spira::kBlock); }
    int resume() const { return progressive ? (sample0 > 0 ? 3 : 1) : 0; }
};

template <class T>
int enqueue_hybrid(Call<T> &k) {
    Ctx &c = k.c;
    const spira_params *p = k.p;
    const spira::Workspace &w = k.plan.ws;
    const uint32_t P = (uint32_t)k.plan.tile_pixels, hblocks = k.plan.blocks(P);
    HIP_TRY(hipMemsetAsync(c.hyb_flags.p, 0, w.hyb_flags, k.st));
    HIP_TRY(hipMemsetAsync(c.accum.p, 0, w.accum, k.st));
    HIP_TRY(hipMemsetAsync(c.hyb_mat.p, 0, w.hyb_mat, k.st));
    HIP_TRY(hipMemsetAsync(c.hyb_state.p, 0, w.hyb_state, k.st));
    hipLaunchKernelGGL(spira::k_hybrid_init, dim3(hblocks), k.block(), 0, k.st, (uint32_t *)c.rng.p, P, k.a.rc.sA, k.a.rc.sB);
    spira::HybridArgs<T> ha{};
    ha.scene = k.a.scene; ha.rc = k.a.rc; ha.state = (T *)c.hyb_state.p; ha.mat = (uint32_t *)c.hyb_mat.p; ha.rng = (uint32_t *)c.rng.p;
    ha.accum = k.accum(); ha.flags = (uint32_t *)c.hyb_flags.p; ha.stats = k.stats();
    for (uint32_t smp = 1; smp <= p->spp; ++smp)
        for (uint32_t ph = 0; ph <= p->max_depth; ++ph) {
            ha.sample = smp; ha.phase = ph;
            if (int rc = launch_lds(spira::k_hybrid<T>, dim3(hblocks), k.block(), k.lds, k.st, ha)) return rc;
        }
    k.launches += 1 + (uint64_t)p->spp * (p->max_depth + 1);
    return 0;
}

template <class T>
int enqueue_metal_wavefront(Call<T> &k) {
    Ctx &c = k.c;
    const spira::Plan &plan = k.plan;
    const dim3 grid(plan.G_metal);
    spira::MetalArgs<T> ma{};
    ma.scene = k.a.scene; ma.rc = k.a.rc;
    ma.ppw = plan.ppw;
    for (int i = 0; i < 2; ++i) { ma.q[i] = k.queue(i); ma.qx[i] = (uint2 *)c.qX[i].p; }
    if (!k.d_rng) k.d_rng = (uint32_t *)c.rng.p;
    ma.L = k.a.L; ma.accum = k.accum(); ma.rng_states = k.d_rng; ma.blk_stats = (uint32_t *)c.blkstats.p;
    ma.resume = k.resume();
    if (int rc = profile_events(c, c.ev_used + 2)) return rc;
    HIP_TRY(hipEventRecord(c.ev_pool[c.ev_used++], k.st));
    ma.stats = k.stats(); ma.redo = nullptr; ma.redo_only = 0;
    if (k.spec) {
        ma.redo = k.redo();
        ma.redo_only = k.spec == 2 ? 2 : 0;
        if (int rc = launch_lds(spira::k_path_metal<T, 2, true>, grid, k.block(), k.lds, k.st, ma)) return rc;
        ma.redo_only = 1;
        ++k.launches;
    }
    if (int rc = plan.R == 2 ? launch_lds(spira::k_path_metal<T, 2, false>, grid, k.block(), k.lds, k.st, ma)
                             : launch_lds(spira::k_path_metal<T, 1, false>, grid, k.block(), k.lds, k.st, ma)) return rc;
    HIP_TRY(hipEventRecord(c.ev_pool[c.ev_used++], k.st));
    hipLaunchKernelGGL(spira::k_fold_stats, dim3(1), dim3(64), 0, k.st, (const uint32_t *)c.blkstats.p, plan.G_metal * plan.wpb, k.stats());
    k.launches += 2;
    k.metal_launches = 1;
    return 0;
}

template <class T>
int enqueue_metal(Call<T> &k) {
    const dim3 grid(k.plan.blocks(k.plan.tile_pixels));
    k.a.pass = 0; k.a.n_first = (uint32_t)k.plan.tile_pixels;
    if (k.spec) {
        if (int rc = launch_lds(spira::k_variant_metal<T, true>, grid, k.block(), k.lds, k.st, k.a, k.accum(), k.d_rng, k.resume(), k.redo(), k.spec == 2 ? 2 : 0)) return rc;
        if (int rc = launch_lds(spira::k_variant_metal<T, false>, grid, k.block(), k.lds, k.st, k.a, k.accum(), k.d_rng, k.resume(), k.redo(), 1)) return rc;
    } else if (int rc = launch_lds(spira::k_variant_metal<T, false>, grid, k.block(), k.lds, k.st, k.a, k.accum(), k.d_rng, k.resume(), (uint32_t *)nullptr, 0))
        return rc;
    k.launches += k.spec ? 2 : 1;
    return 0;
}

template <class T>
int enqueue_cpu_pass(Call<T> &k) {
    const dim3 grid(k.plan.blocks(k.a.n_first));
    if (k.spec) {
        if (int rc = launch_lds(spira::k_variant_cpu<T, true>, grid, k.block(), k.lds, k.st, k.a, k.redo(), k.spec == 2 ? 2 : 0)) return rc;
        if (int rc = launch_lds(spira::k_variant_cpu<T, false>, grid, k.block(), k.lds, k.st, k.a, k.redo(), 1)) return rc;
    } else if (int rc = launch_lds(spira::k_variant_cpu<T, false>, grid, k.block(), k.lds, k.st, k.a, (uint32_t *)nullptr, 0))
        return rc;
    k.launches += k.spec ? 2 : 1;
    return 0;
}

template <class T>
int enqueue_mega_pass(Call<T> &k) {
    const dim3 grid(k.plan.blocks(k.a.n_first));
    const bool ext = (k.p->flags & (SPIRA_EXT_DIELECTRIC | SPIRA_EXT_SPECTRAL)) != 0;
    int rc;
    if (k.a.scene.n_bvh_tris) rc = ext ? launch_lds(spira::k_mega<T, true, true>, grid, k.block(), k.lds, k.st, k.a) : launch_lds(spira::k_mega<T, true, false>, grid, k.block(), k.lds, k.st, k.a);
    else rc = ext ? launch_lds(spira::k_mega<T, false, true>, grid, k.block(), k.lds, k.st, k.a) : launch_lds(spira::k_mega<T, false, false>, grid, k.block(), k.lds, k.st, k.a);
    ++k.launches;
    return rc;
}

template <class T>
int enqueue_path_pass(Call<T> &k, uint32_t *stat_rows) {
    using P4 = typename Call<T>::P4;
    Ctx &c = k.c;
    const spira::Plan &plan = k.plan;
    const spira::Knobs &kn = plan.in.k;
    spira::PathArgs<T> pa{};
    pa.scene = k.a.scene; pa.rc = k.a.rc; pa.L = k.a.L; pa.pass = k.a.pass; pa.n_first = k.a.n_first;
    pa.dense_pct = kn.dense_pct;
    pa.mesh_list = plan.defer_mesh ? (P4 *)c.mesh_list.p : nullptr;
    const spira::Geometry g = plan.geometry(pa.n_first);
    const uint32_t G = g.G;
    pa.cap = g.cap;
    *stat_rows = G * plan.wpb;
    for (int i = 0; i < 2; ++i) {
        pa.q[i] = k.queue(i);
        pa.qref[i] = (uint32_t *)c.qR[i].p;
        pa.qkey[i] = (uint2 *)c.qK[i].p;
    }
    pa.blk_stats = (uint32_t *)c.blkstats.p;
    pa.stats = k.stats();
    if (k.spec) pa.redo = k.redo();
    pa.mesh_mode = 0; pa.mesh_count = nullptr; pa.resume_k = 1; pa.resume_nw = 0;
    pa.mesh_min_batch = kn.mesh_min_batch;
    pa.refill_free = kn.mesh_refill;
    size_t lds_a = k.lds + (size_t)plan.wpb * plan.sub * sizeof(P4) + 128;
    pa.cam_consts = (kn.cam_consts && pa.scene.n_spheres && lds_a + (size_t)pa.scene.n_spheres * sizeof(P4) <= (size_t)160 * 1024) ? 1u : 0u;
    if (pa.cam_consts) lds_a += (size_t)pa.scene.n_spheres * sizeof(P4);
    if (plan.two_pass) {
        pa.mesh_mode = 1; pa.mesh_count = (uint32_t *)c.mesh_count.p;
        pa.resume_nw = G * plan.wpb; pa.resume_k = plan.fat_k(pa.resume_nw);
    }
    if (plan.fused) {
        pa.accum = k.accum(); pa.k_eff = plan.k_eff(pa.pass); pa.fd_keff = spira::fastdiv_make(pa.k_eff);
        pa.accum_first = (pa.pass == 0 && !k.progressive) ? 1u : 0u;
        pa.l_private = plan.l_private ? 1u : 0u;
        pa.sky_runs = plan.sky_runs ? 1u : 0u;
    }
    if (int rc = verify_path_args<T>(c, pa, G)) return rc;
    HIP_TRY(hipEventRecord(c.ev_pool[c.ev_used++], k.st));
    if (int rc = launch_path<T>((int)plan.R, dim3(G), lds_a, k.st, pa, k.spec)) return rc;
    k.launches += k.spec ? 2 : 1;
    if (pa.mesh_mode == 1) {
        if (c.ev_mid.size() <= c.ev_mid_used) {
            hipEvent_t e;
            HIP_TRY(hipEventCreate(&e));
            c.ev_mid.push_back(e); c.ev_mid_end.push_back(0);
        }
        HIP_TRY(hipEventRecord(c.ev_mid[c.ev_mid_used], k.st));
        c.ev_mid_end[c.ev_mid_used++] = c.ev_used;
        spira::PathArgs<T> pb = pa;
        pb.mesh_mode = 2; pb.n_first = 0;
        const uint32_t nwb = pa.resume_nw / pa.resume_k;
        if (int rc = launch_path_resume_entry<T>((int)plan.R, dim3((nwb + plan.wpb - 1) / plan.wpb), lds_a, k.st, pb)) return rc;
        ++k.launches;
    }
    HIP_TRY(hipEventRecord(c.ev_pool[c.ev_used++], k.st));
    return 0;
}

template <class T>
int enqueue_bounce_pass(Call<T> &k, uint32_t *stat_rows) {
    using P4 = typename Call<T>::P4;
    Ctx &c = k.c;
    const spira::Plan &plan = k.plan;
    const spira::Geometry g = plan.geometry(k.a.n_first);
    const size_t nw = (size_t)g.G * plan.wpb;
    k.a.cap = g.cap;
    *stat_rows = k.p->max_depth * g.G * plan.wpb;
    for (uint32_t b = 0; b < k.p->max_depth; ++b) {
        k.a.bounce = b;
        k.a.qout = k.queue(b & 1);
        k.a.qin = k.queue((b & 1) ^ 1);
        k.a.cnt_in = (const uint32_t *)c.counts.p + (size_t)b * nw;
        k.a.cnt_out = (uint32_t *)c.counts.p + (size_t)(b + 1) * nw;
        k.a.blk_stats = (uint32_t *)c.blkstats.p + (size_t)b * nw * 4;
        if (k.profile) HIP_TRY(hipEventRecord(c.ev_pool[c.ev_used++], k.st));
        const size_t lds_b = k.lds + (size_t)plan.wpb * plan.sub * sizeof(P4);
        if (int rc = b == 0 ? launch_bounce<T, true>((int)plan.R, dim3(g.G), lds_b, k.st, k.a) : launch_bounce<T, false>((int)plan.R, dim3(g.G), lds_b, k.st, k.a)) return rc;
        if (k.profile) HIP_TRY(hipEventRecord(c.ev_pool[c.ev_used++], k.st));
        ++k.launches;
    }
    return 0;
}

template <class T>
void enqueue_resolve(Call<T> &k, uint32_t stat_rows) {
    const spira::Plan &plan = k.plan;
    hipLaunchKernelGGL((spira::k_resolve<T>), dim3(plan.blocks(plan.tile_pixels)), k.block(), 0, k.st, k.accum(), (const spira::Pack3<T> *)k.c.L.p,
                       (uint32_t)plan.tile_pixels, plan.k_eff(k.a.pass), (k.a.pass == 0 && !k.progressive) ? 1 : 0,
                       stat_rows ? (const uint32_t *)k.c.blkstats.p : (const uint32_t *)nullptr, stat_rows, k.stats());
    ++k.launches;
}

template <class T>
void enqueue_finalize(Call<T> &k, T *d_hdr, T *d_img) {
    using P4 = typename Call<T>::P4;
    const spira::Plan &plan = k.plan;
    const dim3 grid(plan.blocks(plan.tile_pixels));
    if (k.progressive)
        hipLaunchKernelGGL((spira::k_finalize<T>), grid, k.block(), 0, k.st, (const P4 *)k.accum(), (uint32_t)plan.tile_pixels, 1u, (uint32_t)SPIRA_POST_NONE, d_hdr, (T *)nullptr);
    else
        hipLaunchKernelGGL((spira::k_finalize<T>), grid, k.block(), 0, k.st, (const P4 *)k.accum(), (uint32_t)plan.tile_pixels, k.p->spp,
                           (k.p->flags & SPIRA_SEM_MASK) == SPIRA_SEM_HYBRID ? (uint32_t)SPIRA_POST_NONE : (k.p->flags & SPIRA_POST_MASK), d_hdr, d_img);
    ++k.launches;
}

template <class T>
int prepare_path_call(Call<T> &k, const spira_scene *h, const T *spheres5, const T *materials8, const T *triangles10, const T *camera12, uint32_t rows, bool reuse_scene) {
    Ctx &c = k.c;
    if (int rc = acquire_scene<T>(c, k.st, h, spheres5, materials8, triangles10, k.p, k.a.scene, reuse_scene)) return rc;
    if (int rc = attach_spd<T>(c, k.st, k.p, k.a.scene)) return rc;
    k.spec = k.plan.spec((h ? h->store.moderate : c.scene.moderate) && spira::camera_scale_moderate<T>(camera12));
    fill_const<T>(k.a.rc, camera12, k.p, rows, k.plan.slots);
    if (!fastdiv_selfcheck(k.a.rc.tile_pixels, (uint32_t)k.plan.batch) || !fastdiv_selfcheck(k.a.rc.width, k.a.rc.tile_pixels) ||
        !fastdiv_selfcheck(k.a.rc.stripe_h ? k.a.rc.stripe_h : 1, rows))
        return fail(SPIRA_E_LIMIT, "internal: fast division self-check failed");
    k.a.L = (spira::Pack3<T> *)c.L.p;
    k.a.stats = k.stats();
    k.lds = spira::scene_lds_bytes<T>(k.a.scene.n_spheres, k.a.scene.n_materials, k.a.scene.n_triangles);
    return 0;
}
// ... 2242 lines not shown
int spira_render_multi_scene_f64(const spira_scene *scene, const double cam[12], const spira_params *p, int n_devices, double *out_hdr, double *out_img) {
    if (!scene) return fail(SPIRA_E_INVALID, "scene handle is NULL or was destroyed");
    return render_multi_impl<double>(scene, nullptr, nullptr, nullptr, cam, p, n_devices, out_hdr, out_img);
}
int spira_scene_destroy(spira_scene *scene) {
    if (!scene) return 0;
    if (scene->magic != kSceneMagic) return fail(SPIRA_E_INVALID, "scene handle was already destroyed");
    for (int d = kMaxDevices - 1; d >= 0; --d) {
        spira_scene *h = d ? scene->replica[d] : scene;
        if (!h) continue;
        if (hipSetDevice(h->device) != hipSuccess) return fail(SPIRA_E_HIP, "hipSetDevice failed");
        h->store.release();
        h->magic = 0;
        delete h;
    }
    (void)hipSetDevice(tl_device);
    return 0;
}
int spira_scene_update_f32(spira_scene *scene, const float *spheres5, const float *materials8, const float *triangles10) {
    return scene_update_entry<float>(scene, spheres5, materials8, triangles10, nullptr, false, nullptr);
}
int spira_scene_update_f64(spira_scene *scene, const double *spheres5, const double *materials8, const double *triangles10) {
    return scene_update_entry<double>(scene, spheres5, materials8, triangles10, nullptr, false, nullptr);
}
int spira_scene_update_device_f32(spira_scene *scene, const float *d_triangles10, void *stream) {
    return scene_update_entry<float>(scene, nullptr, nullptr, nullptr, d_triangles10, true, stream);
}
int spira_scene_update_device_f64(spira_scene *scene, const double *d_triangles10, void *stream) {
    return scene_update_entry<double>(scene, nullptr, nullptr, nullptr, d_triangles10, true, stream);
}
int spira_scene_rebuild_f32(spira_scene *scene, const float *triangles10) { return scene_rebuild_entry<float>(scene, triangles10, nullptr, false, nullptr); }
int spira_scene_rebuild_f64(spira_scene *scene, const double *triangles10) { return scene_rebuild_entry<double>(scene, triangles10, nullptr, false, nullptr); }
int spira_scene_rebuild_device_f32(spira_scene *scene, const float *d_triangles10, void *stream) { return scene_rebuild_entry<float>(scene, nullptr, d_triangles10, true, stream); }
int spira_scene_rebuild_device_f64(spira_scene *scene, const double *d_triangles10, void *stream) { return scene_rebuild_entry<double>(scene, nullptr, d_triangles10, true, stream); }
int spira_render_scene_f32(const spira_scene *scene, const float cam[12], const spira_params *p, float *out_hdr, float *out_img) {
    if (!scene) return fail(SPIRA_E_INVALID, "scene handle is NULL or was destroyed");
    return render_entry<float>(scene, nullptr, nullptr, nullptr, cam, p, out_hdr, out_img, false, nullptr);
}
int spira_render_scene_f64(const spira_scene *scene, const double cam[12], const spira_params *p, double *out_hdr, double *out_img) {
    if (!scene) return fail(SPIRA_E_INVALID, "scene handle is NULL or was destroyed");
    return render_entry<double>(scene, nullptr, nullptr, nullptr, cam, p, out_hdr, out_img, false, nullptr);
}
int spira_render_scene_device_f32(const spira_scene *scene, const float cam[12], const spira_params *p, float *d_hdr, float *d_img, void *stream) {
    if (!scene) return fail(SPIRA_E_INVALID, "scene handle is NULL or was destroyed");
    return render_entry<float>(scene, nullptr, nullptr, nullptr, cam, p, d_hdr, d_img, true, stream);
}
int spira_render_scene_device_f64(const spira_scene *scene, const double cam[12], const spira_params *p, double *d_hdr, double *d_img, void *stream) {
    if (!scene) return fail(SPIRA_E_INVALID, "scene handle is NULL or was destroyed");
    return render_entry<double>(scene, nullptr, nullptr, nullptr, cam, p, d_hdr, d_img, true, stream);
}

int spira_render_adaptive_f32(const float *s, const float *m, const float *t, const float cam[12], const spira_params *p, const spira_adaptive *adaptive,
                              float *out_hdr, float *out_img, uint32_t *out_spp, float *out_q) {
    return render_adaptive_entry<float>(nullptr, s, m, t, cam, p, adaptive, out_hdr, out_img, out_spp, out_q, false, nullptr);
}
int spira_render_adaptive_f64(const double *s, const double *m, const double *t, const double cam[12], const spira_params *p, const spira_adaptive *adaptive,
                              double *out_hdr, double *out_img, uint32_t *out_spp, double *out_q) {
    return render_adaptive_entry<double>(nullptr, s, m, t, cam, p, adaptive, out_hdr, out_img, out_spp, out_q, false, nullptr);
}
int spira_render_adaptive_scene_f32(const spira_scene *scene, const float cam[12], const spira_params *p, const spira_adaptive *adaptive,
                                    float *out_hdr, float *out_img, uint32_t *out_spp, float *out_q) {
    if (!scene) return fail(SPIRA_E_INVALID, "scene handle is NULL or was destroyed");
    return render_adaptive_entry<float>(scene, nullptr, nullptr, nullptr, cam, p, adaptive, out_hdr, out_img, out_spp, out_q, false, nullptr);
}
int spira_render_adaptive_scene_f64(const spira_scene *scene, const double cam[12], const spira_params *p, const spira_adaptive *adaptive,
                                    double *out_hdr, double *out_img, uint32_t *out_spp, double *out_q) {
    if (!scene) return fail(SPIRA_E_INVALID, "scene handle is NULL or was destroyed");
    return render_adaptive_entry<double>(scene, nullptr, nullptr, nullptr, cam, p, adaptive, out_hdr, out_img, out_spp, out_q, false, nullptr);
}
int spira_render_adaptive_scene_device_f32(const spira_scene *scene, const float cam[12], const spira_params *p, const spira_adaptive *adaptive,
                                           float *d_hdr, float *d_img, uint32_t *d_spp, float *d_q, void *stream) {
    if (!scene) return fail(SPIRA_E_INVALID, "scene handle is NULL or was destroyed");
    return render_adaptive_entry<float>(scene, nullptr, nullptr, nullptr, cam, p, adaptive, d_hdr, d_img, d_spp, d_q, true, stream);
}
int spira_render_adaptive_scene_device_f64(const spira_scene *scene, const double cam[12], const spira_params *p, const spira_adaptive *adaptive,
                                           double *d_hdr, double *d_img, uint32_t *d_spp, double *d_q, void *stream) {
    if (!scene) return fail(SPIRA_E_INVALID, "scene handle is NULL or was destroyed");
    return render_adaptive_entry<double>(scene, nullptr, nullptr, nullptr, cam, p, adaptive, d_hdr, d_img, d_spp, d_q, true, stream);
}
int spira_sky_pixel_f64(const double cam[12], uint32_t width, uint32_t height, uint32_t i, uint32_t j, const double *spheres5, uint32_t n_spheres) {
    if (!cam || (n_spheres && !spheres5)) return fail(SPIRA_E_INVALID, "cam or spheres5 is NULL");
    return spira::sky_pixel(cam, width, height, i, j, spheres5, n_spheres) ? 1 : 0;
}
int spira_adaptive_converged_f32(const float sum3[3], float q, uint32_t n, double tolerance, double floor) {
    return adaptive_converged_host<float>(sum3, q, n, tolerance, floor);
}
int spira_adaptive_converged_f64(const double sum3[3], double q, uint32_t n, double tolerance, double floor) {
    return adaptive_converged_host<double>(sum3, q, n, tolerance, floor);
}

int spira_render_features_f32(const float *s, const float *m, const float *t, const float cam[12], const spira_params *p,
                              float *out_albedo, float *out_normal, float *out_depth) {
    return features_entry<float>(nullptr, s, m, t, cam, p, out_albedo, out_normal, out_depth, false, nullptr);
}
int spira_render_features_f64(const double *s, const double *m, const double *t, const double cam[12], const spira_params *p,
                              double *out_albedo, double *out_normal, double *out_depth) {
    return features_entry<double>(nullptr, s, m, t, cam, p, out_albedo, out_normal, out_depth, false, nullptr);
}
int spira_render_features_scene_f32(const spira_scene *scene, const float cam[12], const spira_params *p, float *out_albedo, float *out_normal, float *out_depth) {
    if (!scene) return fail(SPIRA_E_INVALID, "scene handle is NULL or was destroyed");
    return features_entry<float>(scene, nullptr, nullptr, nullptr, cam, p, out_albedo, out_normal, out_depth, false, nullptr);
}
int spira_render_features_scene_f64(const spira_scene *scene, const double cam[12], const spira_params *p, double *out_albedo, double *out_normal, double *out_depth) {
    if (!scene) return fail(SPIRA_E_INVALID, "scene handle is NULL or was destroyed");
    return features_entry<double>(scene, nullptr, nullptr, nullptr, cam, p, out_albedo, out_normal, out_depth, false, nullptr);
}
int spira_render_features_scene_device_f32(const spira_scene *scene, const float cam[12], const spira_params *p,
                                           float *d_albedo, float *d_normal, float *d_depth, void *stream) {
    if (!scene) return fail(SPIRA_E_INVALID, "scene handle is NULL or was destroyed");
    return features_entry<float>(scene, nullptr, nullptr, nullptr, cam, p, d_albedo, d_normal, d_depth, true, stream);
}
int spira_render_features_scene_device_f64(const spira_scene *scene, const double cam[12], const spira_params *p,
                                           double *d_albedo, double *d_normal, double *d_depth, void *stream) {
    if (!scene) return fail(SPIRA_E_INVALID, "scene handle is NULL or was destroyed");
    return features_entry<double>(scene, nullptr, nullptr, nullptr, cam, p, d_albedo, d_normal, d_depth, true, stream);
}

int spira_denoise_f32(const float *color, const float *variance, const float *albedo, const float *normal, const float *depth, const spira_denoise *dn,
                      float *out_hdr, float *out_img) {
    return denoise_entry<float>(color, variance, albedo, normal, depth, dn, out_hdr, out_img, false, nullptr);
}
int spira_denoise_f64(const double *color, const double *variance, const double *albedo, const double *normal, const double *depth, const spira_denoise *dn,
                      double *out_hdr, double *out_img) {
    return denoise_entry<double>(color, variance, albedo, normal, depth, dn, out_hdr, out_img, false, nullptr);
}
int spira_denoise_device_f32(const float *d_color, const float *d_variance, const float *d_albedo, const float *d_normal, const float *d_depth, const spira_denoise *dn,
                             float *d_out_hdr, float *d_out_img, void *stream) {
    return denoise_entry<float>(d_color, d_variance, d_albedo, d_normal, d_depth, dn, d_out_hdr, d_out_img, true, stream);
}
int spira_denoise_device_f64(const double *d_color, const double *d_variance, const double *d_albedo, const double *d_normal, const double *d_depth, const spira_denoise *dn,
                             double *d_out_hdr, double *d_out_img, void *stream) {
    return denoise_entry<double>(d_color, d_variance, d_albedo, d_normal, d_depth, dn, d_out_hdr, d_out_img, true, stream);
}

int spira_render_multi_f32(const float *s, const float *m, const float *t, const float cam[12], const spira_params *p, int n_devices,
                           float *out_hdr, float *out_img) {
    return render_multi_impl<float>(nullptr, s, m, t, cam, p, n_devices, out_hdr, out_img);
}
int spira_render_multi_f64(const double *s, const double *m, const double *t, const double cam[12], const spira_params *p, int n_devices,
                           double *out_hdr, double *out_img) {
    return render_multi_impl<double>(nullptr, s, m, t, cam, p, n_devices, out_hdr, out_img);
}

int spira_trace_paths_f32(const float *s, const float *m, const float *t, const float cam[12], const spira_params *p, uint32_t n_paths,
                          const uint32_t *ijs, int *prims, float *ts, float *dirs, float *radiance) {
#ifdef SPIRA_TU_MAIN
    return spira_tu::trace_impl_f32(s, m, t, cam, p, n_paths, ijs, prims, ts, dirs, radiance);
#else
    return trace_impl<float>(s, m, t, cam, p, n_paths, ijs, prims, ts, dirs, radiance);
#endif
}
int spira_trace_paths_f64(const double *s, const double *m, const double *t, const double cam[12], const spira_params *p, uint32_t n_paths,
                          const uint32_t *ijs, int *prims, double *ts, double *dirs, double *radiance) {
    return trace_impl<double>(s, m, t, cam, p, n_paths, ijs, prims, ts, dirs, radiance);
}

int spira_tonemap_f32(float *values, uint64_t n, uint32_t post) {
    if (!values && n) return fail(SPIRA_E_INVALID, "values is NULL");
    post &= SPIRA_POST_MASK;
    for (uint64_t i = 0; i < n; ++i) values[i] = spira::post1<float>(values[i], post);
    return 0;
}

uint32_t spira_stripe_rows(uint32_t height, uint32_t stripe_h, uint32_t stripe_count, uint32_t stripe_rank) {
    if (stripe_count == 0 || stripe_rank >= stripe_count) return 0;
    return stripe_rows(height, stripe_h, stripe_count, stripe_rank);
// ... 5 lines not shown
```

julia-spira_amd/csrc/spira_plan.h:

```cpp
#pragma once
#include <algorithm>
#include <cstddef>
#include <cstdint>

#include "../../include/spira_hip.h"

namespace spira {

struct Knobs {
    uint32_t batch_rays = 160u << 20;
    uint32_t R = 2;
    uint32_t blocks_per_cu = 0;
    uint32_t defer_mesh = 1, mesh_two_pass = 1, fused_resolve = 1, private_l = 1;
    uint32_t spec_div = 1;
    uint32_t dense_pct = 70, mesh_min_batch = 128, mesh_refill = 16, mesh_fat_waves_per_cu = 16, cam_consts = 1;
    uint32_t sky_runs = 1;
};

struct PlanIn {
    uint32_t width = 0, rows = 0;
    uint32_t spp = 0, max_depth = 0, flags = 0, batch_rays = 0;
    uint32_t n_triangles = 0;
    uint32_t num_cus = 0;
    bool progressive = false, caller_rng = false, out_on_device = false;
    bool adaptive = false;
    uint32_t prec = 0, block = 0, waves_per_simd = 0, carry_key = 0;
    uint32_t pack4 = 0, pack3 = 0, pack2 = 0;
    Knobs k;
};

enum class Org { Black, Hybrid, MetalWavefront, Metal, Cpu, Mega, Path, Bounce };

struct Geometry { uint32_t G, cap; };

struct Workspace {
    uint64_t queue4 = 0, queue2 = 0, q_ref = 0, q_key = 0, q_x = 0;
    uint64_t mesh_list = 0, mesh_count = 0, redo = 0, blkstats = 0, L = 0, counts = 0, accum = 0, out_tmp = 0, rng = 0;
    uint64_t hyb_state = 0, hyb_mat = 0, hyb_flags = 0;
};

struct Plan {
    PlanIn in;
    Org org = Org::Black;
    uint32_t R = 2, wpb = 0, sub = 0, max_blocks = 0;
    uint64_t tile_pixels = 0, batch = 0;
    uint32_t slots = 0, n_pass = 0;
    bool mesh_scene = false, defer_mesh = false, two_pass = false;
    bool fused = false, l_private = false;
    bool sky_runs = false;
    bool spec_allowed = false;
    uint32_t G_max = 0, cap_max = 0;
    uint64_t q_rays = 0;
    uint32_t ppw = 0, G_metal = 0;
    Workspace ws;

    Geometry geometry(uint64_t n_first) const {
        if (fused) {
            const uint64_t k = n_first / tile_pixels;
            return {(uint32_t)((tile_pixels + 64 * wpb - 1) / (64 * wpb)), (uint32_t)((64 * k + sub - 1) / sub * sub)};
        }
        const uint64_t n_sub = (n_first + sub - 1) / sub;
        const uint32_t G = (uint32_t)std::min<uint64_t>((n_sub + wpb - 1) / wpb, max_blocks);
        const uint64_t nw = (uint64_t)G * wpb;
        return {G, (uint32_t)(((n_sub + nw - 1) / nw) * sub)};
    }
    uint32_t k_eff(uint32_t pass) const { return std::min(slots, in.spp - pass * slots); }
    uint32_t n_first(uint32_t pass) const { return (uint32_t)((uint64_t)k_eff(pass) * tile_pixels); }
    uint32_t blocks(uint64_t n) const { return (uint32_t)std::min<uint64_t>((n + in.block - 1) / in.block, max_blocks); }
    uint32_t fat_k(uint32_t nw) const {
        const uint32_t fat = std::max<uint32_t>(1, in.num_cus * in.k.mesh_fat_waves_per_cu);
        uint32_t k = 16;
        while (k > 1 && (nw % k != 0 || nw / k < fat)) k >>= 1;
        return k;
    }
    int spec(bool moderate) const {
        uint32_t s = spec_allowed ? in.k.spec_div : 0;
        if (s == 1 && !moderate) s = 0;
        return s > 2 ? 1 : (int)s;
    }
};

inline int sample_range_check(bool progressive, uint32_t sample0, uint32_t spp, const char **msg) {
    if (progressive && (uint64_t)sample0 + spp > SPIRA_MAX_SPP) { *msg = "sample0 + spp exceeds 2^24"; return SPIRA_E_LIMIT; }
    return 0;
}

inline int make_plan(const PlanIn &in, Plan &pl, const char **msg) {
    auto bad = [&](const char *m) { *msg = m; return SPIRA_E_LIMIT; };
    pl = Plan{};
    pl.in = in;
    const Knobs &k = in.k;
    const uint32_t sem = in.flags & SPIRA_SEM_MASK, kern = in.flags & SPIRA_KERNEL_MASK;
    const bool ext = (in.flags & (SPIRA_EXT_DIELECTRIC | SPIRA_EXT_SPECTRAL)) != 0;
    const uint64_t tp = pl.tile_pixels = (uint64_t)in.rows * in.width;
    const uint32_t target = in.batch_rays ? in.batch_rays : k.batch_rays;
    uint64_t slots = std::min<uint64_t>(std::max<uint64_t>(1, target / tp), in.spp);
    const uint64_t n_pass = (in.spp + slots - 1) / slots;
    slots = (in.spp + n_pass - 1) / n_pass;
    if (slots * tp > 0x7FFFFFFFull) return bad("tile too large: rows*width must be < 2^31");
    pl.slots = (uint32_t)slots;
    pl.n_pass = (in.spp + pl.slots - 1) / pl.slots;
    pl.batch = slots * tp;
    pl.org = sem == SPIRA_SEM_HYBRID ? Org::Hybrid : sem == SPIRA_SEM_METAL ? (kern == SPIRA_KERNEL_WAVEFRONT ? Org::MetalWavefront : Org::Metal) :
             sem == SPIRA_SEM_CPU ? Org::Cpu : kern == SPIRA_KERNEL_MEGA ? Org::Mega : kern == SPIRA_KERNEL_BOUNCE ? Org::Bounce : Org::Path;
    const bool persistent = pl.org == Org::Path;
    pl.R = (k.R == 1 && !ext) ? 1 : 2;
    pl.mesh_scene = in.n_triangles > SPIRA_LDS_TRIANGLES;
    pl.defer_mesh = persistent && pl.mesh_scene && in.max_depth <= 128 && k.defer_mesh != 0;
    pl.two_pass = pl.defer_mesh && k.mesh_two_pass != 0;

    const uint32_t blocks_per_cu = k.blocks_per_cu ? k.blocks_per_cu : !persistent ? 16 : (pl.mesh_scene && !pl.two_pass) ? 4 : 32;
    pl.max_blocks = (uint32_t)std::min<uint64_t>((uint64_t)in.num_cus * blocks_per_cu, 0x7FFFFFFFull);
    pl.wpb = in.block / 64;
    pl.sub = 64 * pl.R;
    pl.fused = persistent && in.prec == 8 && pl.R == 2 && in.n_triangles == 0 && !ext && pl.slots <= 64 && k.fused_resolve != 0 && !in.adaptive;
    const Geometry g = pl.geometry(pl.batch);
    pl.G_max = g.G; pl.cap_max = g.cap;
    const uint64_t waves = (uint64_t)g.G * pl.wpb;
    pl.l_private = pl.fused && in.carry_key && in.max_depth <= 128 && k.private_l != 0 && 64ull * waves * pl.slots <= 0x7FFFFFFFull;
    pl.sky_runs = pl.fused && k.sky_runs != 0;
    pl.q_rays = (uint64_t)g.cap * waves;
    if (pl.q_rays > 0xFFFFFFFFull) return bad("pass too large");
    pl.spec_allowed = pl.org == Org::Cpu || (pl.org == Org::Metal && !in.progressive) || (pl.org == Org::MetalWavefront && !in.progressive && pl.R == 2) ||
                      (persistent && pl.R == 2);
    if (in.max_depth == 0) pl.org = Org::Black;

    Workspace &w = pl.ws;
    const uint64_t redo_per_wave = (pl.spec_allowed && k.spec_div) ? sizeof(uint32_t) : 0, stat_row = 4 * sizeof(uint32_t);
    w.accum = tp * in.pack4;
    w.out_tmp = in.out_on_device ? 0 : 2 * 3 * tp * in.prec;
    if (in.caller_rng && !in.out_on_device) w.rng = tp * sizeof(uint32_t);
    switch (pl.org) {
    case Org::Black: break;
    case Org::Hybrid:
        if (tp > 0xFFFFFFFFull / 2) return bad("image too large for SPIRA_SEM_HYBRID");
        w.hyb_state = 12 * tp * in.prec; w.hyb_mat = w.rng = tp * sizeof(uint32_t);
        w.hyb_flags = (uint64_t)in.spp * (in.max_depth + 1) * sizeof(uint32_t);
        break;
    case Org::MetalWavefront: {
        const uint64_t nw0 = (uint64_t)in.num_cus * in.waves_per_simd * pl.wpb;
        pl.ppw = (uint32_t)((((tp + nw0 - 1) / nw0) + 63) / 64 * 64);
        pl.G_metal = (uint32_t)((tp + (uint64_t)pl.ppw * pl.wpb - 1) / ((uint64_t)pl.ppw * pl.wpb));
        const uint64_t nw = (uint64_t)pl.G_metal * pl.wpb, n = nw * pl.ppw;
        w.queue4 = n * in.pack4; w.queue2 = n * in.pack2; w.q_x = n * 2 * sizeof(uint32_t); w.L = n * in.pack3;
        if (!in.caller_rng) w.rng = tp * sizeof(uint32_t);
        w.blkstats = nw * stat_row; w.redo = nw * redo_per_wave;
        break;
    }
    case Org::Metal: case Org::Cpu: case Org::Mega:
        w.L = pl.batch * in.pack3; w.blkstats = waves * stat_row;
        w.redo = (pl.org == Org::Metal ? pl.blocks(tp) : pl.org == Org::Cpu ? pl.max_blocks : 0) * (uint64_t)pl.wpb * redo_per_wave;
        break;
    case Org::Bounce:
        if (in.max_depth > 1) { w.queue4 = pl.q_rays * in.pack4; w.queue2 = pl.q_rays * in.pack2; }
        w.L = pl.batch * in.pack3;
        w.counts = (uint64_t)(in.max_depth + 2) * waves * sizeof(uint32_t); w.blkstats = (uint64_t)(in.max_depth + 1) * waves * stat_row;
        break;
    case Org::Path:
        if (in.max_depth > 1 || pl.mesh_scene) {
            w.queue4 = pl.q_rays * in.pack4; w.queue2 = pl.q_rays * in.pack2;
            if (in.prec == 4) w.q_ref = pl.q_rays * sizeof(uint32_t);
            if (!pl.defer_mesh) w.q_key = pl.q_rays * 2 * sizeof(uint32_t);
        }
        if (pl.defer_mesh) w.mesh_list = 3 * pl.q_rays * in.pack4;
        if (pl.two_pass) w.mesh_count = waves * sizeof(uint32_t);
        w.redo = waves * redo_per_wave; w.blkstats = waves * stat_row;
        w.L = (pl.l_private ? std::max<uint64_t>(pl.batch, 64ull * waves * pl.slots) : pl.batch) * in.pack3;
        break;
    }
    return 0;
}

struct PathLaunch {
    uint32_t blocks = 0, cap = 0, n_first = 0, k_eff = 0;
    uint32_t tile_pixels = 0, max_depth = 0, flags = 0, n_lds_triangles = 0;
    uint32_t mesh_mode = 0, resume_k = 1, resume_nw = 0;
    bool mesh = false, pixel_owning = false, l_private = false;
    uint32_t prec = 0, wpb = 0, carry_key = 0;
};
struct PathNeed {
    uint64_t nw, packets, l_entries;
    bool fits, resume_ok, owning_ok, private_ok;
};
inline PathNeed path_need(const PathLaunch &a) {
    PathNeed n{};
    n.nw = (uint64_t)a.blocks * a.wpb;
    n.packets = n.nw * a.cap;
    n.fits = a.n_first <= n.packets;
    n.resume_ok = a.resume_k != 0 && a.resume_k <= 16 && n.nw % a.resume_k == 0 && a.resume_nw == n.nw;
    n.l_entries = a.l_private ? std::max<uint64_t>(a.n_first, 64ull * n.nw * a.k_eff) : a.n_first;
    const uint64_t tp = a.tile_pixels;
    n.owning_ok = a.prec == 8 && !a.n_lds_triangles && !a.mesh && !(a.flags & (SPIRA_EXT_DIELECTRIC | SPIRA_EXT_SPECTRAL)) && a.k_eff != 0 && a.k_eff <= 64 &&
                  (uint64_t)a.k_eff * tp == a.n_first && 64 * n.nw >= tp && a.cap >= 64ull * a.k_eff;
    n.private_ok = a.pixel_owning && a.carry_key && a.max_depth <= 128 && n.l_entries <= 0x80000000ull;
    return n;
}

struct AdaptiveIn {
    uint32_t min_spp = 0, batch_spp = 0, spp = 0;
    double tolerance = 0, floor = 0;
    uint64_t tile_pixels = 0;
    uint32_t prec = 0, pack3 = 0, num_cus = 0;
};
constexpr uint32_t kAdaptiveItems = 256, kAdaptiveWpb = 4;
struct AdaptiveRound { uint32_t samples, chunk, ppw, grid; uint64_t waves; };
struct AdaptivePlan {
    AdaptiveIn in;
    uint32_t levels = 0;
    uint64_t list_cap = 0;
    uint64_t list_bytes = 0, q_bytes = 0, n_bytes = 0, count_bytes = 0;
    uint64_t lds_round = 0;
    uint32_t level(uint32_t r) const { return (uint32_t)std::min<uint64_t>((uint64_t)in.min_spp + (uint64_t)r * in.batch_spp, in.spp); }
    AdaptiveRound round(uint32_t r, uint64_t n_active) const {
        AdaptiveRound a{};
        a.samples = level(r) - level(r - 1);
        a.chunk = std::min(a.samples, kAdaptiveItems);
        const uint64_t want_waves = std::max<uint64_t>(1, (uint64_t)in.num_cus * 16);
        const uint64_t spread = (n_active + want_waves - 1) / want_waves;
        a.ppw = (uint32_t)std::max<uint64_t>(1, std::min<uint64_t>(std::min<uint32_t>(64, kAdaptiveItems / a.chunk), spread));
        a.waves = (n_active + a.ppw - 1) / a.ppw;
        a.grid = (uint32_t)((a.waves + kAdaptiveWpb - 1) / kAdaptiveWpb);
        return a;
    }
};
inline int adaptive_check(uint32_t min_spp, uint32_t batch_spp, uint32_t spp, double tolerance, double floor, const char **msg) {
    if (min_spp < 2) { *msg = "spira_adaptive: min_spp must be >= 2 (a variance needs two samples)"; return SPIRA_E_INVALID; }
    if (batch_spp < 1) { *msg = "spira_adaptive: batch_spp must be >= 1"; return SPIRA_E_INVALID; }
    if (min_spp > spp) { *msg = "spira_adaptive: min_spp exceeds params->spp (the cap)"; return SPIRA_E_INVALID; }
    if (!(tolerance >= 0) || !(floor >= 0)) { *msg = "spira_adaptive: tolerance and floor must be >= 0"; return SPIRA_E_INVALID; }
    return 0;
}
inline int make_adaptive_plan(const AdaptiveIn &in, AdaptivePlan &ap, const char **msg) {
    ap = AdaptivePlan{};
    ap.in = in;
    if (int rc = adaptive_check(in.min_spp, in.batch_spp, in.spp, in.tolerance, in.floor, msg)) return rc;
    if (in.tile_pixels == 0 || in.tile_pixels > 0x7FFFFFFFull) { *msg = "tile too large: rows*width must be < 2^31"; return SPIRA_E_LIMIT; }
    ap.levels = 1 + (uint32_t)(((uint64_t)(in.spp - in.min_spp) + in.batch_spp - 1) / in.batch_spp);
    ap.list_cap = in.tile_pixels;
    ap.list_bytes = ap.list_cap * sizeof(uint32_t);
    ap.q_bytes = in.tile_pixels * in.prec;
    ap.n_bytes = in.tile_pixels * sizeof(uint32_t);
    ap.count_bytes = 2 * sizeof(uint32_t);
    ap.lds_round = (uint64_t)kAdaptiveWpb * kAdaptiveItems * in.pack3;
    return 0;
}

inline int features_check(uint32_t flags, bool any_output, const char **msg) {
    if (!any_output) { *msg = "all three feature outputs are NULL"; return SPIRA_E_INVALID; }
    if ((flags & SPIRA_SEM_MASK) != SPIRA_SEM_A) { *msg = "feature buffers are built for SPIRA_SEM_A only"; return SPIRA_E_UNSUPPORTED; }
    if ((flags & SPIRA_KERNEL_MASK) != SPIRA_KERNEL_DEFAULT) { *msg = "feature buffers have one kernel organisation: SPIRA_KERNEL_DEFAULT"; return SPIRA_E_UNSUPPORTED; }
    if (flags & (SPIRA_EXT_DIELECTRIC | SPIRA_EXT_SPECTRAL)) { *msg = "SPIRA_EXT_* extensions are not built into the feature kernel"; return SPIRA_E_UNSUPPORTED; }
    return 0;
}
inline uint32_t features_grid(uint64_t tile_pixels, uint32_t block, uint32_t num_cus) {
    const uint64_t cap = std::max<uint64_t>(1, (uint64_t)num_cus * 64);
    return (uint32_t)std::max<uint64_t>(1, std::min<uint64_t>((tile_pixels + block - 1) / block, cap));
}

constexpr uint32_t kDenoiseTileW = 64, kDenoiseTileH = 4, kDenoiseMaxIter = 6;
enum : uint32_t { kDenoiseVariance = 1, kDenoiseAlbedo = 2, kDenoiseNormal = 4, kDenoiseDepth = 8 };
struct DenoiseIn {
    uint32_t width = 0, height = 0, iterations = 0, post = 0;
    double sigma_l = 0, sigma_z = 0;
    uint32_t guides = 0;
    bool want_hdr = false, want_img = false, host = false;
    uint32_t prec = 0, pack4 = 0;
};
struct DenoisePlan {
    DenoiseIn in;
    uint64_t npix = 0;
    uint32_t tiles_x = 0, tiles_y = 0, grid = 0;
    uint32_t grid_flat = 0;
    uint64_t rec_bytes = 0, guide_bytes = 0;
    uint64_t in_planes = 0, out_planes = 0, io_bytes = 0;
    int64_t in_off[5] = {-1, -1, -1, -1, -1};
    uint32_t step(uint32_t it) const { return 1u << it; }
    uint32_t reach(uint32_t it) const { return 2u << it; }
// ... 252 lines not shown
```

julia-spira_amd/csrc/spira_sky.h:

```cpp
#pragma once
#include <stdint.h>
#include "spira_fastdiv.h"

namespace spira {

SPIRA_HD inline bool sky_pixel(const double *cam, uint32_t W, uint32_t H, uint32_t i, uint32_t j, const double *spheres5, uint32_t n_spheres) {
    const double kSlack = 1.0 / 1048576.0, kHuge = 1.0e100, kTiny = 1.0e-100;
    const double w1 = (double)W - 1.0, h1 = (double)H - 1.0;
    const double uc = ((double)i - 0.5) / w1, vc = ((double)j - 0.5) / h1;
    const double hn = __builtin_sqrt((cam[6] * cam[6] + cam[7] * cam[7]) + cam[8] * cam[8]);
    const double vn = __builtin_sqrt((cam[9] * cam[9] + cam[10] * cam[10]) + cam[11] * cam[11]);
    const double rho = (0.5 * (hn / w1 + vn / h1)) * (1.0 + kSlack);
    const double dx = ((cam[3] + cam[6] * uc) + cam[9] * vc) - cam[0];
    const double dy = ((cam[4] + cam[7] * uc) + cam[10] * vc) - cam[1];
    const double dz = ((cam[5] + cam[8] * uc) + cam[11] * vc) - cam[2];
    const double dd = (dx * dx + dy * dy) + dz * dz, dn = __builtin_sqrt(dd);
    if (!(rho >= 0.0 && dn > rho && dn > kTiny && dn < kHuge)) return false;
    const double q = __builtin_sqrt(dd - rho * rho);
    for (uint32_t s = 0; s < n_spheres; ++s) {
        const double *sp = spheres5 + 5 * (uint64_t)s;
        const double r = sp[3];
        const double cx = sp[0] - cam[0], cy = sp[1] - cam[1], cz = sp[2] - cam[2];
        const double cn = __builtin_sqrt((cx * cx + cy * cy) + cz * cz);
        const double xx = cy * dz - cz * dy, xy = cz * dx - cx * dz, xz = cx * dy - cy * dx;
        const double xn = __builtin_sqrt((xx * xx + xy * xy) + xz * xz);
        const double cd = __builtin_fabs((cx * dx + cy * dy) + cz * dz);
        if (!(r > 0.0 && r < kHuge && cn > kTiny && cn < kHuge)) return false;
        if (!(xn * q - cd * rho > (r * (1.0 + kSlack) + cn * kSlack) * dd)) return false;
    }
    return true;
}

}
```

julia-spira_amd/spira_hip/_binding.py:

```python
import ctypes as C
import os
import subprocess

import numpy as np

_HERE = os.path.dirname(os.path.abspath(__file__))
CSRC = os.path.normpath(os.path.join(_HERE, "..", "csrc"))
LIB_PATH = os.environ.get("SPIRA_HIP_LIB", os.path.join(CSRC, "libspira_hip.so"))

ABI_VERSION = 3

SEM_A, SEM_CPU, SEM_METAL, SEM_HYBRID = 0x0, 0x1, 0x2, 0x3
KERNEL_DEFAULT, KERNEL_MEGA, KERNEL_BOUNCE, KERNEL_WAVEFRONT = 0x00, 0x10, 0x20, 0x30
POST_ACES, POST_ACES_GAMMA, POST_CLAMP_GAMMA, POST_NONE = 0x000, 0x100, 0x200, 0x300
ROWS_BOTTOM_UP = 0x1000
FLAG_PROFILE = 0x10000
EXT_DIELECTRIC, EXT_SPECTRAL = 0x20000, 0x40000
MAX_RAYS = 1 << 26
RAY_MISS, RAY_INVALID = -1, -3
CAST_INPLACE = 0x1
MAX_HITS = 16
HITS_COUNT_ALL = 0x2
MAX_NEAR = 16
NEAR_COUNT_ALL = 0x2
MAX_OVERLAP = 16
SDF_SKIPPED = 0xFFFFFFFF
CAM_PINHOLE, CAM_THIN_LENS, CAM_ORTHO = 0, 1, 2
MAX_DEPTH, MAX_SPP = 255, 1 << 24

EXPORTS = [
    "spira_abi_version", "spira_build_id", "spira_last_error", "spira_device_count", "spira_set_device", "spira_get_counters",
    "spira_get_sky_pixels", "spira_sky_pixel_f64",
    "spira_shutdown", "spira_camera_lookat_f32", "spira_camera_lookat_f64", "spira_render_f32", "spira_render_f64",
    "spira_render_device_f32", "spira_render_device_f64", "spira_trace_paths_f32", "spira_trace_paths_f64",
    "spira_tonemap_f32", "spira_stripe_rows", "spira_accumulate_f32", "spira_accumulate_f64", "spira_accumulate_device_f32",
    "spira_accumulate_device_f64", "spira_scene_create_f32", "spira_scene_create_f64", "spira_scene_destroy",
    "spira_render_scene_f32", "spira_render_scene_f64", "spira_render_scene_device_f32", "spira_render_scene_device_f64",
    "spira_render_multi_f32", "spira_render_multi_f64", "spira_scene_create_multi_f32", "spira_scene_create_multi_f64",
    "spira_render_multi_scene_f32", "spira_render_multi_scene_f64",
    "spira_render_adaptive_f32", "spira_render_adaptive_f64", "spira_render_adaptive_scene_f32", "spira_render_adaptive_scene_f64",
    "spira_render_adaptive_scene_device_f32", "spira_render_adaptive_scene_device_f64", "spira_adaptive_converged_f32", "spira_adaptive_converged_f64",
    "spira_render_features_f32", "spira_render_features_f64", "spira_render_features_scene_f32", "spira_render_features_scene_f64",
    "spira_render_features_scene_device_f32", "spira_render_features_scene_device_f64",
    "spira_denoise_f32", "spira_denoise_f64", "spira_denoise_device_f32", "spira_denoise_device_f64",
    "spira_scene_update_f32", "spira_scene_update_f64", "spira_scene_update_device_f32", "spira_scene_update_device_f64",
    "spira_scene_rebuild_f32", "spira_scene_rebuild_f64", "spira_scene_rebuild_device_f32", "spira_scene_rebuild_device_f64",
    "spira_scene_cast_f32", "spira_scene_cast_f64", "spira_scene_cast_device_f32", "spira_scene_cast_device_f64",
    "spira_scene_occluded_f32", "spira_scene_occluded_f64", "spira_scene_occluded_device_f32", "spira_scene_occluded_device_f64",
    "spira_scene_radiance_f32", "spira_scene_radiance_f64", "spira_scene_radiance_device_f32", "spira_scene_radiance_device_f64",
    "spira_camera_rays_f32", "spira_camera_rays_f64", "spira_camera_rays_device_f32", "spira_camera_rays_device_f64",
    "spira_gather_rays_f32", "spira_gather_rays_f64", "spira_gather_rays_device_f32", "spira_gather_rays_device_f64",
    "spira_scene_gather_f32", "spira_scene_gather_f64", "spira_scene_gather_device_f32", "spira_scene_gather_device_f64",
    "spira_scene_gather_visible_f32", "spira_scene_gather_visible_f64", "spira_scene_gather_visible_device_f32", "spira_scene_gather_visible_device_f64",
    "spira_scene_closest_point_f32", "spira_scene_closest_point_f64", "spira_scene_closest_point_device_f32", "spira_scene_closest_point_device_f64",
    "spira_closest_point_triangle_f32", "spira_closest_point_triangle_f64",
    "spira_scene_cast_hits_f32", "spira_scene_cast_hits_f64", "spira_scene_cast_hits_device_f32", "spira_scene_cast_hits_device_f64",
    "spira_scene_nearest_k_f32", "spira_scene_nearest_k_f64", "spira_scene_nearest_k_device_f32", "spira_scene_nearest_k_device_f64",
    "spira_scene_sweep_f32", "spira_scene_sweep_f64", "spira_scene_sweep_device_f32", "spira_scene_sweep_device_f64",
    "spira_scene_sweep_blocked_f32", "spira_scene_sweep_blocked_f64", "spira_scene_sweep_blocked_device_f32", "spira_scene_sweep_blocked_device_f64",
    "spira_sweep_sphere_triangle_f32", "spira_sweep_sphere_triangle_f64",
    "spira_scene_overlap_box_f32", "spira_scene_overlap_box_f64", "spira_scene_overlap_box_device_f32", "spira_scene_overlap_box_device_f64",
    "spira_scene_overlap_any_f32", "spira_scene_overlap_any_f64", "spira_scene_overlap_any_device_f32", "spira_scene_overlap_any_device_f64",
    "spira_overlap_box_triangle_f32", "spira_overlap_box_triangle_f64", "spira_overlap_box_sphere_f32", "spira_overlap_box_sphere_f64",
    "spira_scene_signed_distance_f32", "spira_scene_signed_distance_f64", "spira_scene_signed_distance_device_f32", "spira_scene_signed_distance_device_f64",
]


class SpiraError(RuntimeError):
    pass


class Params(C.Structure):
    _fields_ = [("width", C.c_uint32), ("height", C.c_uint32), ("spp", C.c_uint32), ("max_depth", C.c_uint32),
                ("n_spheres", C.c_uint32), ("n_materials", C.c_uint32), ("n_triangles", C.c_uint32),
                ("flags", C.c_uint32), ("seed", C.c_uint64), ("row0", C.c_uint32), ("rows", C.c_uint32),
                ("stripe_h", C.c_uint32), ("stripe_count", C.c_uint32), ("stripe_rank", C.c_uint32),
                ("batch_rays", C.c_uint32)]


class Counters(C.Structure):
    _fields_ = [("samples", C.c_uint64), ("segments", C.c_uint64), ("rays_enqueued", C.c_uint64),
                ("radiance_rmw", C.c_uint64), ("radiance_stores", C.c_uint64), ("passes", C.c_uint64), ("launches", C.c_uint64),
                ("kernel_ms", C.c_double), ("bounce_kernel_ms", C.c_double), ("bounce_launches", C.c_uint64), ("redone_waves", C.c_uint64), ("rays_parked", C.c_uint64),
                ("mesh_wave_trips", C.c_uint64), ("mesh_lane_trips", C.c_uint64), ("walk_kernel_ms", C.c_double)]

    def as_dict(self):
        return {k: getattr(self, k) for k, _ in self._fields_}


class Adaptive(C.Structure):
    _fields_ = [("min_spp", C.c_uint32), ("batch_spp", C.c_uint32), ("tolerance", C.c_double), ("floor", C.c_double)]


class Denoise(C.Structure):
    _fields_ = [("width", C.c_uint32), ("height", C.c_uint32), ("iterations", C.c_uint32), ("post", C.c_uint32),
                ("sigma_l", C.c_double), ("sigma_z", C.c_double)]


class Radiance(C.Structure):
    _fields_ = [("spp", C.c_uint32), ("max_depth", C.c_uint32), ("flags", C.c_uint32), ("sample0", C.c_uint32),
                ("seed", C.c_uint64), ("key0", C.c_uint32), ("reserved", C.c_uint32)]


class Lens(C.Structure):
    _fields_ = [("model", C.c_uint32), ("width", C.c_uint32), ("height", C.c_uint32), ("sample", C.c_uint32),
                ("seed", C.c_uint64), ("row0", C.c_uint32), ("rows", C.c_uint32), ("lens_radius", C.c_double)]


class GatherVisible(C.Structure):
    _fields_ = [("spp", C.c_uint32), ("sample0", C.c_uint32), ("seed", C.c_uint64), ("key0", C.c_uint32), ("flags", C.c_uint32),
                ("t_min", C.c_double), ("t_max", C.c_double)]


_lib = None

# ... 5 lines not shown
def lib():
    global _lib
    if _lib is None:
        if not os.path.exists(LIB_PATH):
            raise SpiraError("libspira_hip.so is not built (%s); run __graft_entry__.build() / make -C %s" % (LIB_PATH, CSRC))
        try:
            import torch
        except Exception:
            pass
        _lib = C.CDLL(LIB_PATH)
        _lib.spira_last_error.restype = C.c_char_p
        _lib.spira_build_id.restype = C.c_char_p
        _lib.spira_stripe_rows.restype = C.c_uint32
        _lib.spira_stripe_rows.argtypes = [C.c_uint32] * 4
        for name in EXPORTS:
            getattr(_lib, name)
        have = _lib.spira_abi_version()
        if have != ABI_VERSION:
            _lib = None
            raise SpiraError("%s has ABI version %d, this binding was written for %d" % (LIB_PATH, have, ABI_VERSION))
    return _lib


def build_id():
    return lib().spira_build_id().decode()


def _check(rc):
    if rc != 0:
        raise SpiraError("libspira_hip error %d: %s" % (rc, lib().spira_last_error().decode()))


def _dt(prec):
    if prec == "f32":
        return np.float32, C.c_float
    if prec == "f64":
        return np.float64, C.c_double
    raise ValueError("prec must be 'f32' or 'f64'")


def _arr(a, dtype):
    if a is None:
        return None, None
    a = np.ascontiguousarray(a, dtype=dtype)
    return a, a.ctypes.data_as(C.c_void_p)


def make_params(width, height, spp, max_depth, n_spheres, n_materials, n_triangles=0, flags=0, seed=0, row0=0, rows=0,
                stripe_h=0, stripe_count=0, stripe_rank=0, batch_rays=0):
    return Params(width, height, spp, max_depth, n_spheres, n_materials, n_triangles, flags, seed, row0, rows,
                  stripe_h, stripe_count, stripe_rank, batch_rays)


def device_count():
    return lib().spira_device_count()


def set_device(d):
    _check(lib().spira_set_device(C.c_int(d)))


def counters():
    c = Counters()
    _check(lib().spira_get_counters(C.byref(c)))
    d = c.as_dict()
    sky = C.c_uint64(0)
    _check(lib().spira_get_sky_pixels(C.byref(sky)))
    d["sky_pixels"] = sky.value
    return d


def sky_pixel(camera12, width, height, i, j, spheres5):
    cam = np.ascontiguousarray(camera12, dtype=np.float64)
    sp = np.ascontiguousarray(spheres5, dtype=np.float64).reshape(-1, 5)
    assert cam.shape == (12,)
    fn = lib().spira_sky_pixel_f64
    fn.argtypes = [C.c_void_p, C.c_uint32, C.c_uint32, C.c_uint32, C.c_uint32, C.c_void_p, C.c_uint32]
    rc = fn(cam.ctypes.data_as(C.c_void_p), width, height, i, j, sp.ctypes.data_as(C.c_void_p), len(sp))
    if rc < 0:
        _check(rc)
    return rc


def stripe_rows(height, stripe_h, stripe_count, stripe_rank):
    return lib().spira_stripe_rows(height, stripe_h, stripe_count, stripe_rank)


def camera_lookat(position, look_at, up, fov_deg, aspect_ratio, focus_dist=1.0, prec="f32"):
    npdt, cdt = _dt(prec)
    p, pp = _arr(position, npdt)
    l, lp = _arr(look_at, npdt)
    u, up_ = _arr(up, npdt)
    out = np.zeros(12, dtype=npdt)
    if prec == "f32":
        _check(lib().spira_camera_lookat_f32(pp, lp, up_, cdt(fov_deg), cdt(aspect_ratio), out.ctypes.data_as(C.c_void_p)))
    else:
        _check(lib().spira_camera_lookat_f64(pp, lp, up_, cdt(fov_deg), cdt(aspect_ratio), cdt(focus_dist),
                                             out.ctypes.data_as(C.c_void_p)))
    return out


def render(spheres5, materials8, triangles10, camera12, params, prec="f32", want_hdr=True, want_img=False):
    npdt, _ = _dt(prec)
    s, sp = _arr(spheres5, npdt)
    m, mp = _arr(materials8, npdt)
    t, tp = _arr(triangles10, npdt)
    c, cp = _arr(camera12, npdt)
    rows = params.rows if params.rows else params.height
    hdr = np.empty((3, rows, params.width), dtype=npdt) if want_hdr else None
    img = np.empty((3, rows, params.width), dtype=npdt) if want_img else None
    fn = lib().spira_render_f32 if prec == "f32" else lib().spira_render_f64
    _check(fn(sp, mp, tp, cp, C.byref(params), hdr.ctypes.data_as(C.c_void_p) if want_hdr else None,
              img.ctypes.data_as(C.c_void_p) if want_img else None))
    return hdr, img


def render_device(spheres5, materials8, triangles10, camera12, params, d_hdr_ptr, d_img_ptr, stream_ptr, prec="f32"):
    npdt, _ = _dt(prec)
    s, sp = _arr(spheres5, npdt)
    m, mp = _arr(materials8, npdt)
    t, tp = _arr(triangles10, npdt)
    c, cp = _arr(camera12, npdt)
    fn = lib().spira_render_device_f32 if prec == "f32" else lib().spira_render_device_f64
    _check(fn(sp, mp, tp, cp, C.byref(params), C.c_void_p(d_hdr_ptr or None), C.c_void_p(d_img_ptr or None),
              C.c_void_p(stream_ptr or None)))


def render_multi(spheres5, materials8, triangles10, camera12, params, n_devices, prec="f32", want_hdr=True, want_img=False):
    npdt, _ = _dt(prec)
    s, sp = _arr(spheres5, npdt)
    m, mp = _arr(materials8, npdt)
    t, tp = _arr(triangles10, npdt)
    c, cp = _arr(camera12, npdt)
    hdr = np.empty((3, params.height, params.width), dtype=npdt) if want_hdr else None
    img = np.empty((3, params.height, params.width), dtype=npdt) if want_img else None
    fn = lib().spira_render_multi_f32 if prec == "f32" else lib().spira_render_multi_f64
    _check(fn(sp, mp, tp, cp, C.byref(params), C.c_int(n_devices), hdr.ctypes.data_as(C.c_void_p) if want_hdr else None,
              img.ctypes.data_as(C.c_void_p) if want_img else None))
    return hdr, img


class Scene:

    def __init__(self, spheres5, materials8, triangles10=None, prec="f32", n_devices=0):
        npdt, _ = _dt(prec)
        s, sp = _arr(spheres5, npdt)
        m, mp = _arr(materials8, npdt)
        t, tp = _arr(triangles10, npdt)
        self.prec = prec
        self.n_devices = n_devices
        self.counts = (0 if s is None else len(s), len(m), 0 if t is None else len(t))
        self._h = C.c_void_p()
        if n_devices:
            fn = lib().spira_scene_create_multi_f32 if prec == "f32" else lib().spira_scene_create_multi_f64
            _check(fn(sp, mp, tp, C.c_uint32(self.counts[0]), C.c_uint32(self.counts[1]), C.c_uint32(self.counts[2]), C.c_int(n_devices), C.byref(self._h)))
        else:
            fn = lib().spira_scene_create_f32 if prec == "f32" else lib().spira_scene_create_f64
            _check(fn(sp, mp, tp, C.c_uint32(self.counts[0]), C.c_uint32(self.counts[1]), C.c_uint32(self.counts[2]), C.byref(self._h)))

    def render_multi(self, camera12, params, n_devices=None, want_hdr=True, want_img=False):
        npdt, _ = _dt(self.prec)
        c, cp = _arr(camera12, npdt)
        hdr = np.empty((3, params.height, params.width), dtype=npdt) if want_hdr else None
        img = np.empty((3, params.height, params.width), dtype=npdt) if want_img else None
        fn = lib().spira_render_multi_scene_f32 if self.prec == "f32" else lib().spira_render_multi_scene_f64
        _check(fn(self._h, cp, C.byref(params), C.c_int(n_devices or self.n_devices), hdr.ctypes.data_as(C.c_void_p) if want_hdr else None,
# ... 562 lines not shown
```

Measured before the change: 28800.

## Cache per-pixel RNG keys in LDS and cull camera-ray spheres per run

```diff
diff --git a/include/spira_hip.h b/include/spira_hip.h
--- a/include/spira_hip.h
+++ b/include/spira_hip.h
@@ -329,6 +329,7 @@
 int spira_adaptive_converged_f64(const double sum3[3], double q, uint32_t n, double tolerance, double floor);
 
 int spira_sky_pixel_f64(const double camera12[12], uint32_t width, uint32_t height, uint32_t i, uint32_t j, const double *spheres5, uint32_t n_spheres);
+int spira_pixel_reach_f64(const double camera12[12], uint32_t width, uint32_t height, uint32_t i, uint32_t j, const double *spheres5, uint32_t n_spheres, uint32_t *out_mask);
 
 int spira_render_features_f32(const float *spheres5, const float *materials8, const float *triangles10,
                               const float camera12[12], const spira_params *params,
diff --git a/julia-spira_amd/csrc/spira_device.h b/julia-spira_amd/csrc/spira_device.h
--- a/julia-spira_amd/csrc/spira_device.h
+++ b/julia-spira_amd/csrc/spira_device.h
@@ -761,6 +761,47 @@
     }
 }
 
+template <class T, class P>
+__device__ __forceinline__ void closest_hit_cam_masked(const SceneLds<T> &sc, Vec<T> d, T t_min, T &closest, int &prim, P &pol, const Pack4<T> *cam, uint32_t mask) {
+    closest = (T)INFINITY;
+    prim = -1;
+    const T a = dot(d, d);
+    const T two_a = (T)2.0 * a;
+    const T four_a = (T)4 * a;
+    const RootDiv<T> over_2a = root_divisor<T>(two_a, pol);
+    root_t_min<T>(t_min, pol);
+    const uint32_t n = sc.n_spheres;
+    auto from = [&](uint32_t k) -> uint32_t {
+        if (k >= 32u) return k;
+        const uint32_t m = mask >> k;
+        return m ? k + (uint32_t)__builtin_ctz(m) : 32u;
+    };
+    uint32_t s = from(0u);
+    Pack4<T> c_next = cam[s < n ? s : 0u];
+    while (s < n) {
+        const Pack4<T> c = c_next;
+        const uint32_t s_next = from(s + 1u);
+        c_next = cam[s_next < n ? s_next : s];
+        const Vec<T> oc = mk<T>(c.x, c.y, c.z);
+        const T cc = c.w;
+        T b = (T)2.0 * dot(oc, d);
+        const T bb = b * b;
+        T disc = bb - four_a * cc;
+        if (!(disc < 0)) {
+            root_operands<T>(bb, disc, pol);
+            T sq = root_sqrt<T>(disc, pol);
+            T root = root_over<T>(-b - sq, over_2a, pol);
+            bool ok = !(root < t_min || root > closest);
+            if (!ok && root < t_min) {
+                root = root_over<T>(-b + sq, over_2a, pol);
+                ok = !(root < t_min || root > closest);
+            }
+            if (ok) { closest = root; prim = (int)s; }
+        }
+        s = s_next;
+    }
+}
+
 template <class T>
 __device__ __forceinline__ bool mesh_box_hit(const SceneLds<T> &sc, Vec<T> o, Vec<T> d, T closest) {
     const Vec<T> inv = mk<T>(rcp_fast(d.x), rcp_fast(d.y), rcp_fast(d.z));
@@ -1003,6 +1044,23 @@
     rng3<T>(rng_key(rc.sA, rc.sB, pixel, sample, 0), 0, xu, xv, unused);
     T u = pixel_quotient<T>((T)(i - 1) + xu, pd.w1, pol);
     T v = pixel_quotient<T>((T)(j - 1) + xv, pd.h1, pol);
+    o = mk<T>(cam[0], cam[1], cam[2]);
+    const Vec<T> llc = mk<T>(cam[3], cam[4], cam[5]), hor = mk<T>(cam[6], cam[7], cam[8]), ver = mk<T>(cam[9], cam[10], cam[11]);
+    d = normalize(((llc + hor * u) + ver * v) - o, pol);
+}
+
+template <class T, class P>
+__device__ __forceinline__ void camera_ray_lds(const T *cam, const PixelDiv<T> &pd, uint32_t im1, uint32_t jm1, uint32_t hA, uint32_t hB, uint32_t sample,
+                                               Vec<T> &o, Vec<T> &d, P &pol) {
+    T xu, xv, unused;
+    const uint32_t sb = sample << 8;
+    RngKey k;
+    k.hA = mix32(hA ^ sb);
+    k.hB = mix32(hB + sb);
+    k.hBr = (k.hB << 16) | (k.hB >> 16);
+    rng3<T>(k, 0, xu, xv, unused);
+    T u = pixel_quotient<T>((T)im1 + xu, pd.w1, pol);
+    T v = pixel_quotient<T>((T)jm1 + xv, pd.h1, pol);
     o = mk<T>(cam[0], cam[1], cam[2]);
     const Vec<T> llc = mk<T>(cam[3], cam[4], cam[5]), hor = mk<T>(cam[6], cam[7], cam[8]), ver = mk<T>(cam[9], cam[10], cam[11]);
     d = normalize(((llc + hor * u) + ver * v) - o, pol);
@@ -1314,7 +1372,10 @@
     uint32_t accum_first;
     uint32_t l_private;
     uint32_t sky_runs;
+    uint32_t pixel_table, reach_masks;
 };
+struct alignas(16) PixelEntry { uint32_t hA, hB, im1, jm1, pixel, pad[3]; };
+static_assert(sizeof(PixelEntry) == 32, "an entry is 32 bytes (spira_plan.h, kPixelEntryBytes)");
 
 #ifndef SPIRA_RESOLVE_RUN
 #define SPIRA_RESOLVE_RUN 4
@@ -1449,21 +1510,35 @@
     uint32_t sky_mask = 0;
     uint32_t *sky_word = reinterpret_cast<uint32_t *>(cam_lds + 12) + wave;
     static_assert(12 * sizeof(T) + WPB * sizeof(uint32_t) <= 128 || !kOwnT, "a word per wave behind the camera");
+    PixelEntry *own_tab = reinterpret_cast<PixelEntry *>(reinterpret_cast<unsigned char *>(cam_lds) + 128 + (a.cam_consts ? a.scene.n_spheres * sizeof(Pack4<T>) : 0));
+    uint32_t *reach_word = reinterpret_cast<uint32_t *>(own_tab + WPB * 64) + wave * (64 / SPIRA_RESOLVE_RUN);
+    own_tab += wave * 64;
     if constexpr (kOwnT) {
-        if (own && a.sky_runs) {
+        if (own && (a.sky_runs || a.pixel_table || a.reach_masks)) {
             constexpr uint32_t kRun = SPIRA_RESOLVE_RUN, kRuns = 64 / kRun, kRowSlots = 64 / kRun;
             static_assert(kRun == 4 && 2 * 64 * sizeof(Pack3<T>) <= SUB * sizeof(Pack4<T>), "the run mask below is written for runs of 4; a row of terms fits the work list");
             {
                 const uint32_t px = owned_pixel(wid, NW, lane);
                 bool sky = false;
+                uint32_t reach = 0xFFFFFFFFu;
+                uint32_t pi = 1, pj = 1, pixel = 0, sample;
                 if (px < rc.tile_pixels) {
-                    uint32_t pi, pj, pixel, sample;
+                    bool beyond;
                     path_of<T>(rc, px, a.pass, pi, pj, pixel, sample);
-                    sky = sky_pixel(cam_lds, rc.width, rc.height, pi, pj, a.scene.spheres5, a.scene.n_spheres);
+                    reach = pixel_reach(cam_lds, rc.width, rc.height, pi, pj, a.scene.spheres5, a.scene.n_spheres, &beyond);
+                    sky = reach == 0 && !beyond;
+                }
+                if (a.pixel_table) {
+                    PixelEntry &e = own_tab[lane];
+                    e.hA = mix32(rc.sA + pixel); e.hB = mix32(rc.sB ^ pixel); e.im1 = pi - 1; e.jm1 = pj - 1; e.pixel = pixel;
+                }
+                if (a.reach_masks) {
+                    reach |= (uint32_t)__shfl_xor((int)reach, 1); reach |= (uint32_t)__shfl_xor((int)reach, 2);
+                    if (lane % kRun == 0) reach_word[lane / kRun] = reach;
                 }
                 unsigned long long b = __ballot(sky);
                 b &= b >> 1; b &= b >> 2;
-                for (uint32_t g = 0; g < kRuns; ++g) sky_mask |= (uint32_t)((b >> (kRun * g)) & 1ull) << g;
+                if (a.sky_runs) for (uint32_t g = 0; g < kRuns; ++g) sky_mask |= (uint32_t)((b >> (kRun * g)) & 1ull) << g;
             }
             Pack3<T> *s_sky = reinterpret_cast<Pack3<T> *>(s_rnd);
             for (uint32_t m = sky_mask; m; m &= m - 1u) {
@@ -1551,10 +1626,12 @@
                 bool parked = false; T park_t = 0; int park_prim = -1;
                 uint32_t qf = idx;
                 bool in = idx < limit;
+                uint32_t own_l = 0, own_slot = 0;
                 if (own && first) {
                     const uint32_t t = idx / SPIRA_RESOLVE_RUN, run = fastdiv(t, a.fd_keff);
-                    const uint32_t px = owned_pixel(wid, NW, run * SPIRA_RESOLVE_RUN + idx % SPIRA_RESOLVE_RUN);
-                    qf = (t - run * a.k_eff) * rc.tile_pixels + px;
+                    own_l = run * SPIRA_RESOLVE_RUN + idx % SPIRA_RESOLVE_RUN; own_slot = t - run * a.k_eff;
+                    const uint32_t px = owned_pixel(wid, NW, own_l);
+                    qf = own_slot * rc.tile_pixels + px;
                     in = in && px < rc.tile_pixels;
                     if constexpr (kOwnT) in = in && !((*sky_word >> run) & 1u);
                 }
@@ -1564,9 +1641,26 @@
                         uint32_t pixel, sample, pi, pj;
                         Vec<T> d;
                         q[r] = ql;
-                        path_of<T>(rc, qf, a.pass, pi, pj, pixel, sample);
-                        if (kCarry) { ka[r] = mix32(rc.sA + pixel) ^ (sample << 8); kb[r] = mix32(rc.sB ^ pixel) + (sample << 8); }
-                        camera_ray_lds<T>(rc, cam_lds, pix_div, pi, pj, pixel, sample, o[r], d, pol);
+                        uint32_t cmask = 0xFFFFFFFFu;
+                        if constexpr (kOwnT) {
+                            uint32_t hA, hB, im1, jm1;
+                            if (own && a.pixel_table) {
+                                const PixelEntry e = own_tab[own_l];
+                                hA = e.hA; hB = e.hB; im1 = e.im1; jm1 = e.jm1;
+                                sample = rc.sample0 + a.pass * rc.slots + own_slot;
+                            } else {
+                                path_of<T>(rc, qf, a.pass, pi, pj, pixel, sample);
+                                hA = mix32(rc.sA + pixel); hB = mix32(rc.sB ^ pixel); im1 = pi - 1; jm1 = pj - 1;
+                            }
+                            ka[r] = hA ^ (sample << 8); kb[r] = hB + (sample << 8);
+                            camera_ray_lds<T>(cam_lds, pix_div, im1, jm1, hA, hB, sample, o[r], d, pol);
+                            if (own && a.reach_masks && a.k_eff % (64 / SPIRA_RESOLVE_RUN) == 0 && sc.n_spheres <= 32u)
+                                cmask = (uint32_t)__builtin_amdgcn_readfirstlane((int)reach_word[fastdiv((sub * SUB + r * 64) / SPIRA_RESOLVE_RUN, a.fd_keff)]);
+                        } else {
+                            path_of<T>(rc, qf, a.pass, pi, pj, pixel, sample);
+                            if (kCarry) { ka[r] = mix32(rc.sA + pixel) ^ (sample << 8); kb[r] = mix32(rc.sB ^ pixel) + (sample << 8); }
+                            camera_ray_lds<T>(rc, cam_lds, pix_div, pi, pj, pixel, sample, o[r], d, pol);
+                        }
                         if (EXT) { ex[r].flags = rc.flags; if (rc.flags & kExtSpectral) beta[r] = ext_wavelength<T>(sc, rc.sA, rc.sB, pixel, sample, ex[r]); }
                         T t; uint32_t slot = 0;
                         int prim;
@@ -1574,7 +1668,10 @@
                             if (kCam && a.cam_consts) closest_hit_local<T, Pol, TRI, true>(sc, o[r], d, (T)0.001, t, prim, pol, cam_sph);
                             else closest_hit_local<T, Pol, TRI>(sc, o[r], d, (T)0.001, t, prim, pol);
                             parked = mesh_box_hit<T>(sc, o[r], d, t);
-                        } else if (kCam && !BVH && a.cam_consts) { closest_hit_local<T, Pol, TRI, true>(sc, o[r], d, (T)0.001, t, prim, pol, cam_sph); }
+                        } else if (kCam && !BVH && a.cam_consts) {
+                            if constexpr (kOwnT) closest_hit_cam_masked<T, Pol>(sc, d, (T)0.001, t, prim, pol, cam_sph, cmask);
+                            else closest_hit_local<T, Pol, TRI, true>(sc, o[r], d, (T)0.001, t, prim, pol, cam_sph);
+                        }
                         else prim = closest_hit<T, BVH, Pol, TRI>(sc, o[r], d, (T)0.001, t, slot, pol);
                         ++n_seg;
                         if (parked) { park_t = t; park_prim = prim; pend[r].v = d; }
@@ -1969,11 +2066,10 @@
             else resolve_pixel<T>(a.accum, a.L, rc.tile_pixels, a.k_eff, a.accum_first != 0, px);
         }
         const uint32_t seg = __shfl(n_seg, 0), rmw = __shfl(n_rmw, 0), sto = __shfl(n_store, 0);
-        if (lane < 4) {
-            unsigned long long *f = lane == 0 ? &a.stats->segments : (lane == 1 ? &a.stats->rays_enqueued : (lane == 2 ? &a.stats->radiance_rmw : &a.stats->radiance_store));
-            atomicAdd(f, (unsigned long long)(lane == 0 ? seg : (lane == 1 ? n_enq : (lane == 2 ? rmw : sto))));
-        }
-        if constexpr (kOwnT) if (lane == 4 && sky_mask) atomicAdd(&a.stats->sky_pixels, (unsigned long long)(SPIRA_RESOLVE_RUN * __popc(sky_mask)));
+        if (lane < 4 || (kOwnT && lane == 4 && sky_mask)) {
+            unsigned long long *f = lane == 0 ? &a.stats->segments : (lane == 1 ? &a.stats->rays_enqueued : (lane == 2 ? &a.stats->radiance_rmw : (lane == 3 ? &a.stats->radiance_store : &a.stats->sky_pixels)));
+            atomicAdd(f, (unsigned long long)(lane == 0 ? seg : (lane == 1 ? n_enq : (lane == 2 ? rmw : (lane == 3 ? sto : SPIRA_RESOLVE_RUN * (uint32_t)__popc(sky_mask))))));
+        }
     }
     MESH_STAT(if (lane == 0) { unsigned long long *g = g_mesh_dbg + (mesh_mode == 2u ? 16 : 0);
                                atomicAdd(&g[0], __builtin_readcyclecounter() - dbg_t0); atomicAdd(&g[1], dbg_sess); atomicAdd(&g[2], (unsigned long long)dbg_ns);
diff --git a/julia-spira_amd/csrc/spira_hip.hip b/julia-spira_amd/csrc/spira_hip.hip
--- a/julia-spira_amd/csrc/spira_hip.hip
+++ b/julia-spira_amd/csrc/spira_hip.hip
@@ -690,6 +690,7 @@
     k.mesh_fat_waves_per_cu = env_u32("SPIRA_MESH_FAT_WAVES_PER_CU", 16);
     k.cam_consts = env_u32("SPIRA_CAM_CONSTS", 1);
     k.sky_runs = env_u32("SPIRA_SKY_RUNS", 1);
+    k.pixel_table = env_u32("SPIRA_PIXEL_TABLE", 1); k.reach_masks = env_u32("SPIRA_REACH_MASKS", 1);
     return k;
 }
 template <class T>
@@ -722,8 +723,9 @@
     return 0;
 }
 
-template <class T>
-int verify_path_args(const Ctx &c, const spira::PathArgs<T> &a, uint32_t first_launch_blocks) {
+static_assert(sizeof(spira::PixelEntry) == spira::kPixelEntryBytes && spira::kOwnRuns * SPIRA_RESOLVE_RUN == 64, "own_lds_bytes sizes what k_path's prologue writes");
+template <class T>
+int verify_path_args(const Ctx &c, const spira::PathArgs<T> &a, uint32_t first_launch_blocks, size_t own_lds = 0) {
     using P4 = spira::Pack4<T>;
     using P2 = spira::Pack2<T>;
     spira::PathLaunch l;
@@ -732,6 +734,7 @@
     l.mesh_mode = a.mesh_mode; l.resume_k = a.resume_k; l.resume_nw = a.resume_nw;
     l.mesh = a.scene.n_bvh_tris != 0; l.pixel_owning = a.accum != nullptr; l.l_private = a.l_private != 0;
     l.prec = sizeof(T); l.wpb = spira::kBlock / 64; l.carry_key = SPIRA_CARRY_KEY;
+    l.pixel_table = a.pixel_table != 0; l.reach_masks = a.reach_masks != 0; l.own_lds = own_lds;
     const spira::PathNeed need = spira::path_need(l);
     const uint64_t nw = need.nw, n = need.packets;
     auto covers = [](const DevBuf &b, const void *ptr, uint64_t bytes) { return ptr == b.p && b.p != nullptr && b.cap >= bytes; };
@@ -750,6 +753,7 @@
     if (!bad && !covers(c.stats, a.stats, sizeof(spira::Stats))) bad = "counters";
     if (!bad && a.accum && (!covers(c.accum, a.accum, (uint64_t)a.rc.tile_pixels * sizeof(P4)) || !need.owning_ok)) bad = "pixel-owning pass";
     if (!bad && a.l_private && !need.private_ok) bad = "wave-private radiance blocks";
+    if (!bad && !need.table_ok) bad = "pixel table and reach masks in LDS";
     if (bad) return fail(SPIRA_E_LIMIT, std::string("internal: a workspace is smaller than the launch needs (") + bad + ")");
     return 0;
 }
@@ -911,6 +915,7 @@
     size_t lds_a = k.lds + (size_t)plan.wpb * plan.sub * sizeof(P4) + 128;
     pa.cam_consts = (kn.cam_consts && pa.scene.n_spheres && lds_a + (size_t)pa.scene.n_spheres * sizeof(P4) <= (size_t)160 * 1024) ? 1u : 0u;
     if (pa.cam_consts) lds_a += (size_t)pa.scene.n_spheres * sizeof(P4);
+    size_t own_lds = 0;
     if (plan.two_pass) {
         pa.mesh_mode = 1; pa.mesh_count = (uint32_t *)c.mesh_count.p;
         pa.resume_nw = G * plan.wpb; pa.resume_k = plan.fat_k(pa.resume_nw);
@@ -920,8 +925,13 @@
         pa.accum_first = (pa.pass == 0 && !k.progressive) ? 1u : 0u;
         pa.l_private = plan.l_private ? 1u : 0u;
         pa.sky_runs = plan.sky_runs ? 1u : 0u;
-    }
-    if (int rc = verify_path_args<T>(c, pa, G)) return rc;
+        if ((plan.pixel_table || plan.reach_masks) && lds_a + spira::own_lds_bytes(plan.wpb) <= (size_t)160 * 1024) {
+            own_lds = (size_t)spira::own_lds_bytes(plan.wpb);
+            lds_a += own_lds;
+            pa.pixel_table = plan.pixel_table ? 1u : 0u; pa.reach_masks = plan.reach_masks ? 1u : 0u;
+        }
+    }
+    if (int rc = verify_path_args<T>(c, pa, G, own_lds)) return rc;
     HIP_TRY(hipEventRecord(c.ev_pool[c.ev_used++], k.st));
     if (int rc = launch_path<T>((int)plan.R, dim3(G), lds_a, k.st, pa, k.spec)) return rc;
     k.launches += k.spec ? 2 : 1;
@@ -3330,6 +3340,11 @@
     if (!cam || (n_spheres && !spheres5)) return fail(SPIRA_E_INVALID, "cam or spheres5 is NULL");
     return spira::sky_pixel(cam, width, height, i, j, spheres5, n_spheres) ? 1 : 0;
 }
+int spira_pixel_reach_f64(const double cam[12], uint32_t width, uint32_t height, uint32_t i, uint32_t j, const double *spheres5, uint32_t n_spheres, uint32_t *out_mask) {
+    if (!cam || !out_mask || (n_spheres && !spheres5)) return fail(SPIRA_E_INVALID, "cam, out_mask or spheres5 is NULL");
+    *out_mask = spira::pixel_reach(cam, width, height, i, j, spheres5, n_spheres);
+    return 0;
+}
 int spira_adaptive_converged_f32(const float sum3[3], float q, uint32_t n, double tolerance, double floor) {
     return adaptive_converged_host<float>(sum3, q, n, tolerance, floor);
 }
diff --git a/julia-spira_amd/csrc/spira_plan.h b/julia-spira_amd/csrc/spira_plan.h
--- a/julia-spira_amd/csrc/spira_plan.h
+++ b/julia-spira_amd/csrc/spira_plan.h
@@ -15,6 +15,8 @@
     uint32_t spec_div = 1;
     uint32_t dense_pct = 70, mesh_min_batch = 128, mesh_refill = 16, mesh_fat_waves_per_cu = 16, cam_consts = 1;
     uint32_t sky_runs = 1;
+    uint32_t pixel_table = 1;
+    uint32_t reach_masks = 1;
 };
 
 struct PlanIn {
@@ -48,6 +50,7 @@
     bool mesh_scene = false, defer_mesh = false, two_pass = false;
     bool fused = false, l_private = false;
     bool sky_runs = false;
+    bool pixel_table = false, reach_masks = false;
     bool spec_allowed = false;
     uint32_t G_max = 0, cap_max = 0;
     uint64_t q_rays = 0;
@@ -119,6 +122,8 @@
     const uint64_t waves = (uint64_t)g.G * pl.wpb;
     pl.l_private = pl.fused && in.carry_key && in.max_depth <= 128 && k.private_l != 0 && 64ull * waves * pl.slots <= 0x7FFFFFFFull;
     pl.sky_runs = pl.fused && k.sky_runs != 0;
+    pl.pixel_table = pl.fused && k.pixel_table != 0;
+    pl.reach_masks = pl.fused && k.reach_masks != 0;
     pl.q_rays = (uint64_t)g.cap * waves;
     if (pl.q_rays > 0xFFFFFFFFull) return bad("pass too large");
     pl.spec_allowed = pl.org == Org::Cpu || (pl.org == Org::Metal && !in.progressive) || (pl.org == Org::MetalWavefront && !in.progressive && pl.R == 2) ||
@@ -171,16 +176,20 @@
     return 0;
 }
 
+constexpr uint32_t kPixelEntryBytes = 32, kOwnRuns = 16;
+inline uint64_t own_lds_bytes(uint32_t wpb) { return (uint64_t)wpb * (64 * kPixelEntryBytes + kOwnRuns * sizeof(uint32_t)); }
 struct PathLaunch {
     uint32_t blocks = 0, cap = 0, n_first = 0, k_eff = 0;
     uint32_t tile_pixels = 0, max_depth = 0, flags = 0, n_lds_triangles = 0;
     uint32_t mesh_mode = 0, resume_k = 1, resume_nw = 0;
     bool mesh = false, pixel_owning = false, l_private = false;
+    bool pixel_table = false, reach_masks = false;
+    uint64_t own_lds = 0;
     uint32_t prec = 0, wpb = 0, carry_key = 0;
 };
 struct PathNeed {
     uint64_t nw, packets, l_entries;
-    bool fits, resume_ok, owning_ok, private_ok;
+    bool fits, resume_ok, owning_ok, private_ok, table_ok;
 };
 inline PathNeed path_need(const PathLaunch &a) {
     PathNeed n{};
@@ -193,6 +202,7 @@
     n.owning_ok = a.prec == 8 && !a.n_lds_triangles && !a.mesh && !(a.flags & (SPIRA_EXT_DIELECTRIC | SPIRA_EXT_SPECTRAL)) && a.k_eff != 0 && a.k_eff <= 64 &&
                   (uint64_t)a.k_eff * tp == a.n_first && 64 * n.nw >= tp && a.cap >= 64ull * a.k_eff;
     n.private_ok = a.pixel_owning && a.carry_key && a.max_depth <= 128 && n.l_entries <= 0x80000000ull;
+    n.table_ok = (!a.pixel_table && !a.reach_masks) || (a.pixel_owning && a.own_lds >= own_lds_bytes(a.wpb));
     return n;
 }
 
diff --git a/julia-spira_amd/csrc/spira_sky.h b/julia-spira_amd/csrc/spira_sky.h
--- a/julia-spira_amd/csrc/spira_sky.h
+++ b/julia-spira_amd/csrc/spira_sky.h
@@ -4,7 +4,7 @@
 
 namespace spira {
 
-SPIRA_HD inline bool sky_pixel(const double *cam, uint32_t W, uint32_t H, uint32_t i, uint32_t j, const double *spheres5, uint32_t n_spheres) {
+SPIRA_HD inline uint32_t pixel_reach(const double *cam, uint32_t W, uint32_t H, uint32_t i, uint32_t j, const double *spheres5, uint32_t n_spheres, bool *beyond = nullptr) {
     const double kSlack = 1.0 / 1048576.0, kHuge = 1.0e100, kTiny = 1.0e-100;
     const double w1 = (double)W - 1.0, h1 = (double)H - 1.0;
     const double uc = ((double)i - 0.5) / w1, vc = ((double)j - 0.5) / h1;
@@ -15,8 +15,10 @@
     const double dy = ((cam[4] + cam[7] * uc) + cam[10] * vc) - cam[1];
     const double dz = ((cam[5] + cam[8] * uc) + cam[11] * vc) - cam[2];
     const double dd = (dx * dx + dy * dy) + dz * dz, dn = __builtin_sqrt(dd);
-    if (!(rho >= 0.0 && dn > rho && dn > kTiny && dn < kHuge)) return false;
+    if (!(rho >= 0.0 && dn > rho && dn > kTiny && dn < kHuge)) { if (beyond) *beyond = n_spheres > 32u; return 0xFFFFFFFFu; }
     const double q = __builtin_sqrt(dd - rho * rho);
+    uint32_t reach = 0;
+    bool far = false;
     for (uint32_t s = 0; s < n_spheres; ++s) {
         const double *sp = spheres5 + 5 * (uint64_t)s;
         const double r = sp[3];
@@ -25,10 +27,16 @@
         const double xx = cy * dz - cz * dy, xy = cz * dx - cx * dz, xz = cx * dy - cy * dx;
         const double xn = __builtin_sqrt((xx * xx + xy * xy) + xz * xz);
         const double cd = __builtin_fabs((cx * dx + cy * dy) + cz * dz);
-        if (!(r > 0.0 && r < kHuge && cn > kTiny && cn < kHuge)) return false;
-        if (!(xn * q - cd * rho > (r * (1.0 + kSlack) + cn * kSlack) * dd)) return false;
+        const bool missed = (r > 0.0 && r < kHuge && cn > kTiny && cn < kHuge) && (xn * q - cd * rho > (r * (1.0 + kSlack) + cn * kSlack) * dd);
+        if (!missed) { if (s < 32u) reach |= 1u << s; else far = true; }
     }
-    return true;
+    if (beyond) *beyond = far;
+    return reach;
+}
+
+SPIRA_HD inline bool sky_pixel(const double *cam, uint32_t W, uint32_t H, uint32_t i, uint32_t j, const double *spheres5, uint32_t n_spheres) {
+    bool beyond = false;
+    return pixel_reach(cam, W, H, i, j, spheres5, n_spheres, &beyond) == 0 && !beyond;
 }
 
 }
diff --git a/julia-spira_amd/spira_hip/_binding.py b/julia-spira_amd/spira_hip/_binding.py
--- a/julia-spira_amd/spira_hip/_binding.py
+++ b/julia-spira_amd/spira_hip/_binding.py
@@ -30,7 +30,7 @@
 
 EXPORTS = [
     "spira_abi_version", "spira_build_id", "spira_last_error", "spira_device_count", "spira_set_device", "spira_get_counters",
-    "spira_get_sky_pixels", "spira_sky_pixel_f64",
+    "spira_get_sky_pixels", "spira_sky_pixel_f64", "spira_pixel_reach_f64",
     "spira_shutdown", "spira_camera_lookat_f32", "spira_camera_lookat_f64", "spira_render_f32", "spira_render_f64",
     "spira_render_device_f32", "spira_render_device_f64", "spira_trace_paths_f32", "spira_trace_paths_f64",
     "spira_tonemap_f32", "spira_stripe_rows", "spira_accumulate_f32", "spira_accumulate_f64", "spira_accumulate_device_f32",
@@ -202,6 +202,17 @@
     return rc
 
 
+def pixel_reach(camera12, width, height, i, j, spheres5):
+    cam = np.ascontiguousarray(camera12, dtype=np.float64)
+    sp = np.ascontiguousarray(spheres5, dtype=np.float64).reshape(-1, 5)
+    assert cam.shape == (12,)
+    fn = lib().spira_pixel_reach_f64
+    fn.argtypes = [C.c_void_p, C.c_uint32, C.c_uint32, C.c_uint32, C.c_uint32, C.c_void_p, C.c_uint32, C.c_void_p]
+    mask = C.c_uint32(0)
+    _check(fn(cam.ctypes.data_as(C.c_void_p), width, height, i, j, sp.ctypes.data_as(C.c_void_p), len(sp), C.byref(mask)))
+    return mask.value
+
+
 def stripe_rows(height, stripe_h, stripe_count, stripe_rank):
     return lib().spira_stripe_rows(height, stripe_h, stripe_count, stripe_rank)
 
```

After: 29720 (median of 6 runs). +3.2%, better.
